# akuhara/RF_INV

Hardware: NVIDIA B200
Metric: forward+likelihood evals/sec (higher is better)
Workload: dtype f64

## Files before the change

### rf_inv_b200/csrc/forward.cu

```cuda
#include <cstdlib>
#include "rfinv_common.cuh"

#if defined(RFINV_PHASE_TIMING) && !defined(RFINV_FWD_GENERAL_TU)
__device__ unsigned long long g_phase[16];
#define PHASE_MARK(i)                                                            \
  do {                                                                           \
    if (tid == 0) {                                                              \
      const long long now__ = clock64();                                         \
      atomicAdd(&g_phase[i], (unsigned long long)(now__ - t_phase__));           \
      t_phase__ = now__;                                                         \
    }                                                                            \
  } while (0)
#define PHASE_INIT() long long t_phase__ = clock64(); if (tid == 0) atomicAdd(&g_phase[15], 1ULL)
extern "C" int rfinv_debug_get_phases(unsigned long long* out) {
  cudaError_t e = cudaMemcpyFromSymbol(out, g_phase, sizeof(g_phase));
  unsigned long long zero[16] = {0};
  cudaMemcpyToSymbol(g_phase, zero, sizeof(zero));
  return e == cudaSuccess ? 0 : 2;
}
#define PREP_MARK(i)                                                             \
  do {                                                                           \
    if (lane == 0) {                                                             \
      const long long now__ = clock64();                                         \
      atomicAdd(&g_phase[8 + (i)], (unsigned long long)(now__ - tp_phase__));    \
      tp_phase__ = now__;                                                        \
    }                                                                            \
  } while (0)
#define PREP_INIT() long long tp_phase__ = clock64()
#else
#define PHASE_MARK(i) do { } while (0)
#define PHASE_INIT() do { } while (0)
#define PREP_MARK(i) do { } while (0)
#define PREP_INIT() do { } while (0)
#endif

namespace {

struct LayerConst {
  double c1x, s1x, c1e, s1e;
  double c16x, s16x, c16e, s16e;
  double cbx, sbx, cbe, sbe;
  double t12, t21;
  double u11, u12, u21, u22;
  double cb2x, cb2e;
};
constexpr int LC_DOUBLES = sizeof(LayerConst) / sizeof(double);
static_assert(LC_DOUBLES % 2 == 0, "LayerConst is moved in 16-byte pieces");

struct TraceSel {
  int n;
  unsigned long long packed;
  __host__ __device__ int t(int i) const { return (int)((packed >> (4 * i)) & 15ULL); }
  __host__ void push(int trace) { packed |= (unsigned long long)trace << (4 * n); ++n; }
};
static_assert(RFINV_MAX_TRC <= 16, "TraceSel packs trace indices in four bits");

struct RayConst {
  double h14[4], h23[4];
  double a1, b1;
  double q1a, q1b, q2a, q2b;
  double thw, cbw, sbw;
  double wseed[4];
  double tp;
  double2 edge[4];
  double sta[4];
  int k, valid;
  int npre, l_sta;
};
constexpr int RC_DOUBLES = sizeof(RayConst) / sizeof(double);
static_assert(sizeof(RayConst) % 16 == 0, "RayConst is moved in 16-byte pieces");

__device__ __forceinline__ void rot(double& c, double& s, double cb, double sb) {
  double c2 = c * cb - s * sb;
  double s2 = s * cb + c * sb;
  c = c2;
  s = s2;
}

struct Wave { double a1, a2, b1, b2; };

__device__ __forceinline__ void wave_rotate(Wave& w, double c1, double s1, double c2, double s2) {
  const double a1 = fma(-s1, w.a2, c1 * w.a1);
  const double a2 = fma(s1, w.a1, c1 * w.a2);
  const double b1 = fma(-s2, w.b2, c2 * w.b1);
  const double b2 = fma(s2, w.b1, c2 * w.b2);
  w.a1 = a1; w.a2 = a2; w.b1 = b1; w.b2 = b2;
}

__device__ __forceinline__ void wave_interface(Wave& w, double t12, double t21, double u11, double u12, double u21,
                                               double u22) {
  const double a1 = fma(t12, w.b1, w.a1);
  const double b1 = fma(t21, w.a1, w.b1);
  const double a2 = fma(u12, w.b2, u11 * w.a2);
  const double b2 = fma(u22, w.b2, u21 * w.a2);
  w.a1 = a1; w.a2 = a2; w.b1 = b1; w.b2 = b2;
}

__device__ __forceinline__ double2 cmul(double2 a, double2 b) {
  return make_double2(a.x * b.x - a.y * b.y, a.x * b.y + a.y * b.x);
}

__device__ __forceinline__ void surface_response(const double* h14, const double* h23, const Wave& wa, const Wave& wb,
                                                 double cw, int ipha, double2& fr, double2& fv, double gain = 1.0) {
  const double2 A3 = make_double2(fma(h14[0], wa.a1, h14[1] * wa.b1), fma(h23[0], wa.a2, h23[1] * wa.b2));
  const double2 A4 = make_double2(fma(h14[2], wa.a1, h14[3] * wa.b1), fma(h23[2], wa.a2, h23[3] * wa.b2));
  const double2 B3 = make_double2(fma(h14[0], wb.a1, h14[1] * wb.b1), fma(h23[0], wb.a2, h23[1] * wb.b2));
  const double2 B4 = make_double2(fma(h14[2], wb.a1, h14[3] * wb.b1), fma(h23[2], wb.a2, h23[3] * wb.b2));
  const double2 p = cmul(A3, B4), q = cmul(B3, A4);
  const double2 dl = make_double2(p.x - q.x, p.y - q.y);
  const double rn = gain / (dl.x * dl.x + dl.y * dl.y);
  const double2 inv = make_double2(dl.x * rn, -dl.y * rn);
  double2 ur, uz;
  if (ipha >= 0) {
    ur = cmul(B4, inv);
    const double2 w = cmul(A4, inv);
    uz = make_double2(w.y * cw, -w.x * cw);
  } else {
    const double2 w0 = cmul(B3, inv);
    ur = make_double2(-w0.x, -w0.y);
    const double2 w = cmul(A3, inv);
    uz = make_double2(-w.y * cw, w.x * cw);
  }
  fr = make_double2(ur.x, -ur.y);
  fv = make_double2(-uz.x, uz.y);
}

__device__ __forceinline__ void surface_response_buried(const double* h14, const double* h23, const Wave& wa, const Wave& wb,
                                                        int ipha, double2 ya, double2 yb, double2& fr, double2& fv) {
  const double2 A3 = make_double2(fma(h14[0], wa.a1, h14[1] * wa.b1), fma(h23[0], wa.a2, h23[1] * wa.b2));
  const double2 A4 = make_double2(fma(h14[2], wa.a1, h14[3] * wa.b1), fma(h23[2], wa.a2, h23[3] * wa.b2));
  const double2 B3 = make_double2(fma(h14[0], wb.a1, h14[1] * wb.b1), fma(h23[0], wb.a2, h23[1] * wb.b2));
  const double2 B4 = make_double2(fma(h14[2], wb.a1, h14[3] * wb.b1), fma(h23[2], wb.a2, h23[3] * wb.b2));
  const double2 p = cmul(A3, B4), q = cmul(B3, A4);
  const double2 dl = make_double2(p.x - q.x, p.y - q.y);
  const double rn = 1.0 / (dl.x * dl.x + dl.y * dl.y);
  const double2 inv = make_double2(dl.x * rn, -dl.y * rn);
  double2 al, be;
  if (ipha >= 0) {
    al = cmul(B4, inv);
    const double2 w = cmul(A4, inv);
    be = make_double2(-w.x, -w.y);
  } else {
    const double2 w0 = cmul(B3, inv);
    al = make_double2(-w0.x, -w0.y);
    be = cmul(A3, inv);
  }
  const double2 ur = make_double2(fma(al.x, ya.x, be.x * yb.x), fma(al.y, ya.x, be.y * yb.x));
  const double2 s = make_double2(fma(al.x, ya.y, be.x * yb.y), fma(al.y, ya.y, be.y * yb.y));
  const double2 uz = make_double2(-s.y, s.x);
  fr = make_double2(ur.x, -ur.y);
  fv = make_double2(-uz.x, uz.y);
}

__device__ __forceinline__ void mat2_mul(const double* a, const double* b, double* c) {
  const double c0 = fma(a[0], b[0], a[1] * b[2]), c1 = fma(a[0], b[1], a[1] * b[3]);
  const double c2 = fma(a[2], b[0], a[3] * b[2]), c3 = fma(a[2], b[1], a[3] * b[3]);
  c[0] = c0; c[1] = c1; c[2] = c2; c[3] = c3;
}

struct PrepBasis {
  double v14[4], v23[4];
  double i14[4], i23[4];
};
struct PrepSerial {
  double tr[8];
  double ic[6];
  double tpterm, pad;
};
struct PrepShared {
  double h, rho, irho, beta2, inv_b2, inv_a2, a, b;
};
constexpr int PB_DOUBLES = sizeof(PrepBasis) / sizeof(double), PS_DOUBLES = sizeof(PrepSerial) / sizeof(double);
constexpr int PSH_DOUBLES = sizeof(PrepShared) / sizeof(double);
constexpr int PREP_RAYS_PER_PASS = 6;
constexpr int PREP_MISC_DOUBLES = 8;
__host__ __device__ inline size_t prep_sorted_doubles(int km) { return ((size_t)3 * km + 1) & ~(size_t)1; }
__host__ __device__ inline size_t prep_smem_model_doubles(int km) { return prep_sorted_doubles(km) + (size_t)(km + 2) * PSH_DOUBLES + PREP_MISC_DOUBLES; }
__host__ __device__ inline size_t prep_smem_ray_doubles(int km) { return (size_t)(km + 1) * PB_DOUBLES + (size_t)km * PS_DOUBLES + RC_DOUBLES + 8; }

__device__ __forceinline__ void small_sincos(double x, double* sn, double* cs) {
  if (fabs(x) < 0.01) {
    const double x2 = x * x;
    *cs = fma(x2, fma(x2, fma(x2, -1.0 / 720.0, 1.0 / 24.0), -0.5), 1.0);
    *sn = x * fma(x2, fma(x2, fma(x2, -1.0 / 5040.0, 1.0 / 120.0), -1.0 / 6.0), 1.0);
  } else {
    sincos(x, sn, cs);
  }
}

__device__ __forceinline__ double warp_scan_mul(double x, int lane) {
#pragma unroll
  for (int o = 1; o < 32; o <<= 1) {
    const double y = __shfl_up_sync(0xffffffffu, x, o);
    if (lane >= o) x *= y;
  }
  return x;
}

template <bool BURIED, bool HOSTLAYOUT>
__global__ void __maxnreg__(80) prep_kernel(const DevConfig cfg, const ModelBatch mb, double* __restrict__ lc_out,
                                                                 double* __restrict__ rc_out, uint8_t* __restrict__ is_valid,
                                                                 int* __restrict__ counter, int n_models, int ntr_eff, int nthr_fwd,
                                                                 int rays_per_cta, int m_begin) {
  extern __shared__ __align__(16) double prep_smem[];
  const int warp = threadIdx.x >> 5, lane = threadIdx.x & 31;
  const int n_groups = (ntr_eff + rays_per_cta - 1) / rays_per_cta;
  const int bm = blockIdx.x / n_groups, t_first = (blockIdx.x - bm * n_groups) * rays_per_cta;
  const int ci = m_begin + bm;
  const int nr_cta = min(rays_per_cta, ntr_eff - t_first);
  pdl_trigger();
  if (blockIdx.x == 0 && m_begin == 0 && threadIdx.x < RFINV_MAX_TRC) counter[threadIdx.x] = 0;
  if (ci >= n_models) return;
  if (mb.n_active_dev && ci >= *mb.n_active_dev) return;
  const int c = mb.active ? mb.active[ci] : ci;
  const int km = cfg.k_max, C = mb.C;
  const bool has_ray = warp < nr_cta;
  const int t0 = t_first + (has_ray ? warp : 0);
  const size_t item = (size_t)ci * ntr_eff + t0;
  double* zs = prep_smem;
  double *dps = zs + km, *dss = dps + km;
  PrepShared* LA = reinterpret_cast<PrepShared*>(zs + prep_sorted_doubles(km));
  double* s_misc = reinterpret_cast<double*>(LA + km + 2);
  int* s_int = reinterpret_cast<int*>(s_misc + 1);
  double* ray0 = s_misc + PREP_MISC_DOUBLES;
  const size_t ray_stride = prep_smem_ray_doubles(km);
  auto ray_basis = [&](int t) { return reinterpret_cast<PrepBasis*>(ray0 + (size_t)t * ray_stride); };
  auto ray_serial = [&](int t) { return reinterpret_cast<PrepSerial*>(ray0 + (size_t)t * ray_stride + (size_t)(km + 1) * PB_DOUBLES); };
  auto ray_const = [&](int t) { return reinterpret_cast<RayConst*>(ray0 + (size_t)t * ray_stride + (size_t)(km + 1) * PB_DOUBLES + (size_t)km * PS_DOUBLES); };
  auto ray_water = [&](int t) { return reinterpret_cast<double*>(ray_const(t)) + RC_DOUBLES; };
  constexpr bool buried = BURIED;

  PREP_INIT();
  if (warp == 0) {
    int k = mb.k[c];
    double zr[2] = {0.0, 0.0}, dr[2] = {0.0, 0.0}, sr[2] = {0.0, 0.0};
    static_assert(RFINV_MAX_K <= 64, "two elements per lane");
#pragma unroll
    for (int q = 0; q < 2; ++q) {
      const int i = lane + 32 * q;
      if (i < km - 1) {
        if (HOSTLAYOUT) {
          zr[q] = mb.z[(size_t)c * (km - 1) + i]; sr[q] = mb.dvs[(size_t)c * km + i];
          if (cfg.vp_mode == 1) dr[q] = mb.dvp[(size_t)c * km + i];
        } else {
          zr[q] = mb.z[(size_t)i * C + c]; dr[q] = mb.dvp[(size_t)i * C + c]; sr[q] = mb.dvs[(size_t)i * C + c];
        }
      }
    }
    double dvs_half, dvp_half = 0.0;
    if (HOSTLAYOUT) { dvs_half = mb.dvs[(size_t)c * km + km - 1]; if (cfg.vp_mode == 1) dvp_half = mb.dvp[(size_t)c * km + km - 1]; }
    else { dvs_half = mb.dvs[(size_t)(km - 1) * C + c]; dvp_half = mb.dvp[(size_t)(km - 1) * C + c]; }
    k = k < 1 ? 1 : (k > km - 1 ? km - 1 : k);
    double* zu = reinterpret_cast<double*>(ray_basis(0));
    double *du = zu + km, *su = du + km;
#pragma unroll
    for (int q = 0; q < 2; ++q) {
      const int i = lane + 32 * q;
      if (i < k) { zu[i] = zr[q]; du[i] = dr[q]; su[i] = sr[q]; }
    }
    __syncwarp();
    for (int i = lane; i < k; i += 32) {
      const double zi = zu[i];
      int rank = 0;
      for (int j = 0; j < k; ++j) { const double zj = zu[j]; rank += (zj < zi || (zj == zi && j < i)) ? 1 : 0; }
      zs[rank] = zi; dps[rank] = du[i]; dss[rank] = su[i];
    }
    __syncwarp();

    int ls = -1;
    double h_part = 0.0;
    if (buried) {
      double z_tmp = 0.0;
      ls = k;
      for (int l = 0; l < k; ++l) {
        const double hl = l == 0 ? __dsub_rn(zs[0], cfg.sdep) : __dsub_rn(zs[l], zs[l - 1]);
        z_tmp = __dadd_rn(z_tmp, hl);
        if (!(z_tmp < cfg.bdep)) { ls = l; h_part = __dsub_rn(__dadd_rn(cfg.bdep, hl), z_tmp); break; }
      }
      if (ls == k) h_part = __dsub_rn(cfg.bdep, z_tmp);
    }
    const int ka = buried ? k + 1 : k;
    PREP_MARK(0);
    bool valid = true;
    for (int la = lane; la <= ka; la += 32) {
      const int l = (buried && la > ls) ? la - 1 : la;
      double zc, h, dvs_l, dvp_l;
      if (l == 0) { zc = __dmul_rn(0.5, __dadd_rn(cfg.sdep, zs[0])); h = __dsub_rn(zs[0], cfg.sdep); dvs_l = dss[0]; dvp_l = dps[0]; }
      else if (l < k) { zc = __dmul_rn(0.5, __dadd_rn(zs[l], zs[l - 1])); h = __dsub_rn(zs[l], zs[l - 1]); dvs_l = dss[l]; dvp_l = dps[l]; }
      else { zc = __dmul_rn(0.5, __dadd_rn(cfg.z_max, zs[k - 1])); h = 999.0; dvs_l = dvs_half; dvp_l = dvp_half; }
      double a, b;
      bool ok = layer_velocity(cfg, zc, dvs_l, dvp_l, a, b);
      if (l == 0) ok = ok && !(h < __dmul_rn(0.125, a));
      else if (l < k) ok = ok && !(h < cfg.h_min);
      valid = valid && ok;
      if (buried) {
        if (la == ls) h = h_part;
        else if (la == ls + 1 && ls < k) h = __dsub_rn(h, h_part);
      }
      PrepShared S;
      S.h = h; S.a = a; S.b = b;
      S.rho = vp_to_rho(a);
      S.irho = 1.0 / S.rho;
      S.beta2 = __dmul_rn(b, b);
      S.inv_b2 = __ddiv_rn(1.0, S.beta2);
      S.inv_a2 = __ddiv_rn(1.0, __dmul_rn(a, a));
      LA[la] = S;
    }
    valid = __all_sync(0xffffffffu, valid);
    if (lane == 0) { s_int[0] = k; s_int[1] = ls; s_int[2] = valid ? 1 : 0; s_misc[0] = h_part; }
    PREP_MARK(1);
  }
  __syncthreads();

  const int k = s_int[0], ls = s_int[1];
  const bool valid = s_int[2] != 0;
  const int ka = buried ? k + 1 : k;
  const int kb = (buried && ls == k) ? k : ka;
  PrepBasis* PB = ray_basis(warp);
  PrepSerial* PS = ray_serial(warp);
  if (has_ray) {

  const double p = cfg.rayp[t0];
  const int ipha = cfg.ipha[t0];
  const double p2 = __dmul_rn(p, p);
  const double nyq = (double)(cfg.nfft / 2);
  int nyq_doublings = 0;
  while ((nthr_fwd << nyq_doublings) < cfg.nfft_p2 / 2) ++nyq_doublings;
  for (int la = lane; la <= ka; la += 32) {
    const PrepShared S = LA[la];
    const double h = S.h, rho = S.rho, beta2 = S.beta2;
    double tp_sign = 1.0;
    if (buried) {
      if (la == ls) tp_sign = ls == k ? -1.0 : 0.0;
      else if (la < ls) tp_sign = 0.0;
    }
    const double bp = 1.0 - 2.0 * beta2 * p2;
    const double eta = sqrt(__dsub_rn(S.inv_b2, p2));
    const double xi = sqrt(__dsub_rn(S.inv_a2, p2));
    if (la < ka) {
      PrepBasis& Q = PB[la];
      PrepSerial& Z = PS[la];
      const double g2 = 2.0 * beta2 * p;
      const double ieta = 1.0 / eta, irho = S.irho, ixi = 1.0 / xi;
      Q.v14[0] = p; Q.v14[1] = 1.0; Q.v14[2] = rho * bp; Q.v14[3] = -rho * g2;
      Q.v23[0] = xi; Q.v23[1] = -p * ieta; Q.v23[2] = -rho * g2 * xi; Q.v23[3] = -rho * bp * ieta;
      Q.i14[0] = g2; Q.i14[1] = irho; Q.i14[2] = bp; Q.i14[3] = -p * irho;
      Q.i23[0] = bp * ixi; Q.i23[1] = -p * irho * ixi; Q.i23[2] = -g2 * eta; Q.i23[3] = -eta * irho;
      Z.tpterm = cfg.deconv_mode == 0 ? __dmul_rn(tp_sign, __dmul_rn(h, ipha == 1 ? xi : eta)) : 0.0;
      LayerConst* L = reinterpret_cast<LayerConst*>(lc_out) + item * km + la;
      const double thx = cfg.domg * xi * h, the = cfg.domg * eta * h;
      double snx, csx, sne, cse;
      sincos(thx, &snx, &csx); L->c1x = csx; L->s1x = snx;
      sincos(the, &sne, &cse); L->c1e = cse; L->s1e = sne;
#pragma unroll
      for (int d = 0; d < 4; ++d) {
        const double c2 = fma(csx, csx, -snx * snx), s2 = 2.0 * csx * snx; csx = c2; snx = s2;
        const double c3 = fma(cse, cse, -sne * sne), s3 = 2.0 * cse * sne; cse = c3; sne = s3;
      }
      L->c16x = csx; L->s16x = snx; L->c16e = cse; L->s16e = sne;
      for (int b = 16; b < nthr_fwd; b <<= 1) {
        const double c2 = fma(csx, csx, -snx * snx), s2 = 2.0 * csx * snx; csx = c2; snx = s2;
        const double c3 = fma(cse, cse, -sne * sne), s3 = 2.0 * cse * sne; cse = c3; sne = s3;
      }
      L->cbx = csx; L->sbx = snx; L->cbe = cse; L->sbe = sne;
      L->cb2x = csx + csx; L->cb2e = cse + cse;
      small_sincos((double)1.0e-5f * xi * h, &Z.tr[1], &Z.tr[0]);
      small_sincos((double)1.0e-5f * eta * h, &Z.tr[3], &Z.tr[2]);
      double cn = csx, sn2 = snx, ce = cse, se = sne;
      if (cfg.fft_general) {
        sincos(nyq * thx, &sn2, &cn);
        sincos(nyq * the, &se, &ce);
      } else {
        for (int d = 0; d < nyq_doublings; ++d) {
          const double c2 = fma(cn, cn, -sn2 * sn2), s2 = 2.0 * cn * sn2; cn = c2; sn2 = s2;
          const double c3 = fma(ce, ce, -se * se), s3 = 2.0 * ce * se; ce = c3; se = s3;
        }
      }
      Z.tr[4] = cn; Z.tr[5] = sn2; Z.tr[6] = ce; Z.tr[7] = se;
    } else {
      double* W = ray_water(warp);
      W[4] = xi; W[5] = eta; W[6] = bp;
    }
  }
  __syncwarp();

  PREP_MARK(2);
  double carryP = 1.0, carryS = 1.0;
  double sP_last = 1.0, sS_last = 1.0;
  double sP_sta = 1.0, sS_sta = 1.0;
  for (int base = 0; base < ka; base += 32) {
    const int l = base + lane;
    double t14[4] = {1.0, 0.0, 0.0, 1.0}, t23[4] = {1.0, 0.0, 0.0, 1.0};
    if (l >= 1 && l < ka) {
      mat2_mul(PB[l].i14, PB[l - 1].v14, t14);
      mat2_mul(PB[l].i23, PB[l - 1].v23, t23);
    }
    const double sP = carryP * warp_scan_mul(t14[0], lane), sS = carryS * warp_scan_mul(t14[3], lane);
    double sPp = __shfl_up_sync(0xffffffffu, sP, 1), sSp = __shfl_up_sync(0xffffffffu, sS, 1);
    if (lane == 0) { sPp = carryP; sSp = carryS; }
    if (l >= 1 && l < ka) {
      double* ic = PS[l - 1].ic;
      const double rP = 1.0 / sP, rS = 1.0 / sS;
      const double pp = sPp * rP, sp = sSp * rP, ps = sPp * rS, ss = sSp * rS;
      ic[0] = t14[1] * sp; ic[1] = t14[2] * ps;
      ic[2] = t23[0] * pp; ic[3] = t23[1] * sp; ic[4] = t23[2] * ps; ic[5] = t23[3] * ss;
      LayerConst* L = reinterpret_cast<LayerConst*>(lc_out) + item * km + (l - 1);
      L->t12 = ic[0]; L->t21 = ic[1]; L->u11 = ic[2]; L->u12 = ic[3]; L->u21 = ic[4]; L->u22 = ic[5];
    }
    const int last_lane = (ka - 1 - base) < 31 ? (ka - 1 - base) : 31;
    if (buried && ls >= base && ls < base + 32) { sP_sta = __shfl_sync(0xffffffffu, sP, ls - base); sS_sta = __shfl_sync(0xffffffffu, sS, ls - base); }
    if (kb - 1 >= base && kb - 1 < base + 32) { sP_last = __shfl_sync(0xffffffffu, sP, kb - 1 - base); sS_last = __shfl_sync(0xffffffffu, sS, kb - 1 - base); }
    carryP = __shfl_sync(0xffffffffu, sP, last_lane);
    carryS = __shfl_sync(0xffffffffu, sS, last_lane);
  }
  if (lane == 0) {
    LayerConst* L = reinterpret_cast<LayerConst*>(lc_out) + item * km + (ka - 1);
    L->t12 = 0.0; L->t21 = 0.0; L->u11 = 1.0; L->u12 = 0.0; L->u21 = 0.0; L->u22 = 1.0;
    double* ic = PS[ka - 1].ic;
    ic[0] = 0.0; ic[1] = 0.0; ic[2] = 1.0; ic[3] = 0.0; ic[4] = 0.0; ic[5] = 1.0;
  }
  __syncwarp();

  PREP_MARK(3);
  {
    RayConst R;
    double cw0 = 1.0, sw0 = 0.0, cw1 = 1.0, sw1 = 0.0, rw = 0.0;
    if (cfg.sdep > 0.0) {
      const double aw = 1.5, rhow = 1.0, hw = cfg.sdep;
      const double xiw = sqrt(1.0 / (aw * aw) - p * p);
      R.thw = cfg.domg * xiw * hw;
      sincos(R.thw, &R.wseed[1], &R.wseed[0]);
      R.cbw = R.wseed[0]; R.sbw = R.wseed[1];
#pragma unroll
      for (int d = 0; d < 4; ++d) { const double c2 = fma(R.cbw, R.cbw, -R.sbw * R.sbw), s2 = 2.0 * R.cbw * R.sbw; R.cbw = c2; R.sbw = s2; }
      R.wseed[2] = R.cbw; R.wseed[3] = R.sbw;
      for (int b = 16; b < nthr_fwd; b <<= 1) { const double c2 = fma(R.cbw, R.cbw, -R.sbw * R.sbw), s2 = 2.0 * R.cbw * R.sbw; R.cbw = c2; R.sbw = s2; }
      rw = rhow / xiw;
      small_sincos((double)1.0e-5f * xiw * hw, &sw0, &cw0);
      sincos(nyq * R.thw, &sw1, &cw1);
    } else {
      R.thw = 0.0; R.cbw = 1.0; R.sbw = 0.0;
      R.wseed[0] = R.wseed[2] = 1.0; R.wseed[1] = R.wseed[3] = 0.0;
    }
    {
      const PrepShared& H = LA[ka];
      const double* W = ray_water(warp);
      const double a = H.a, b = H.b, rho = H.rho, beta2 = H.beta2, xi = W[4], eta = W[5], bp = W[6];
      const double r1 = 1.0 / (2.0 * rho * a * xi), r2 = 1.0 / (2.0 * rho * b * eta);
      const double e11 = beta2 * p * (2.0 * rho * xi) * r1, e12 = bp * rho * r1, e13 = p * r1, e14 = xi * r1;
      const double e21 = bp * rho * r2, e22 = b * p, e23 = eta * r2, e24 = p * r2;
      const double r14[4] = {e11, e14, e21, -e24};
      const double r23[4] = {-e12, e13, e22, e23};
      const PrepBasis& Q = PB[kb - 1];
      const double v14[4] = {Q.v14[0] * sP_last, Q.v14[1] * sS_last, Q.v14[2] * sP_last, Q.v14[3] * sS_last};
      const double v23[4] = {Q.v23[0] * sP_last, Q.v23[1] * sS_last, Q.v23[2] * sP_last, Q.v23[3] * sS_last};
      mat2_mul(r14, v14, R.h14);
      mat2_mul(r23, v23, R.h23);
    }
    {
      const PrepBasis& Q = PB[0];
      R.a1 = Q.i14[0]; R.b1 = Q.i14[2];
      R.q1a = -rw * Q.i14[1]; R.q1b = -rw * Q.i14[3];
      R.q2a = Q.i23[0]; R.q2b = Q.i23[2];
    }
    R.l_sta = -1;
    R.sta[0] = R.sta[1] = R.sta[2] = R.sta[3] = 0.0;
    if (buried) {
      const PrepBasis& Q = PB[ls];
      R.l_sta = ls;
      R.sta[0] = Q.v14[0] * sP_sta; R.sta[1] = Q.v14[1] * sS_sta;
      R.sta[2] = Q.v23[0] * sP_sta; R.sta[3] = Q.v23[1] * sS_sta;
    }
    R.k = kb;
    R.valid = valid;
    R.tp = 0.0; R.npre = 0;
#pragma unroll
    for (int i = 0; i < 4; ++i) R.edge[i] = make_double2(0.0, 0.0);
    if (lane == 0) {
      *ray_const(warp) = R;
      double* W = ray_water(warp);
      W[0] = cw0; W[1] = sw0; W[2] = cw1; W[3] = sw1;
    }
  }
  PREP_MARK(4);
  }
  __syncthreads();

  for (int r0 = warp * PREP_RAYS_PER_PASS; r0 < nr_cta; r0 += (int)(blockDim.x >> 5) * PREP_RAYS_PER_PASS) {
    const int nr = min(PREP_RAYS_PER_PASS, nr_cta - r0);
    const bool vec_lane = lane < 4 * nr, tp_lane = lane >= 4 * nr && lane < 5 * nr;
    const int tr_ray = r0 + (vec_lane ? (lane >> 2) : (tp_lane ? lane - 4 * nr : 0));
    const RayConst* Rr = ray_const(tr_ray);
    const double* Wr = ray_water(tr_ray);
    const PrepSerial* Zr = ray_serial(tr_ray);
    const bool is_b = lane & 1, is_nyq = (lane >> 1) & 1;
    Wave w;
    double2 y_sta = make_double2(0.0, 0.0);
    double tp = 0.0;
    {
      const double cw = is_nyq ? Wr[2] : Wr[0], sw = is_nyq ? Wr[3] : Wr[1];
      if (!is_b) { w.a1 = Rr->a1; w.b1 = Rr->b1; w.a2 = 0.0; w.b2 = 0.0; }
      else { w.a1 = sw * Rr->q1a; w.b1 = sw * Rr->q1b; w.a2 = cw * Rr->q2a; w.b2 = cw * Rr->q2b; }
    }
    if (vec_lane) {
      const int o = is_nyq ? 4 : 0;
      const double st0 = Rr->sta[0], st1 = Rr->sta[1], st2 = Rr->sta[2], st3 = Rr->sta[3];
      Wave w_bc = w;
      for (int l = 0; l < ka; ++l) {
        const PrepSerial& Q = Zr[l];
        wave_rotate(w, Q.tr[o], Q.tr[o + 1], Q.tr[o + 2], Q.tr[o + 3]);
        if (buried && l == ls) { y_sta.x = fma(st0, w.a1, st1 * w.b1); y_sta.y = fma(st2, w.a2, st3 * w.b2); }
        if (l == kb - 1) w_bc = w;
        if (l + 1 < ka) wave_interface(w, Q.ic[0], Q.ic[1], Q.ic[2], Q.ic[3], Q.ic[4], Q.ic[5]);
      }
      w = w_bc;
    } else if (tp_lane) {
      for (int l = 0; l < ka; ++l) tp = __dadd_rn(tp, Zr[l].tpterm);
      RayConst* Rw = ray_const(tr_ray);
      const int iph = cfg.ipha[t_first + tr_ray];
      Rw->tp = tp;
      Rw->npre = iph == 1 ? f_nint((-cfg.t_start - tp) / cfg.delta)
                          : f_nint((-cfg.t_start + tp) / cfg.delta);
    }
    PREP_MARK(5);
    {
      const int rr = lane >> 1, e = lane & 1;
      const bool fin = lane < 2 * nr;
      const int src_a = fin ? 4 * rr + 2 * e : 0, src_b = src_a + 1;
      Wave ea, eb;
      ea.a1 = __shfl_sync(0xffffffffu, w.a1, src_a); ea.a2 = __shfl_sync(0xffffffffu, w.a2, src_a);
      ea.b1 = __shfl_sync(0xffffffffu, w.b1, src_a); ea.b2 = __shfl_sync(0xffffffffu, w.b2, src_a);
      eb.a1 = __shfl_sync(0xffffffffu, w.a1, src_b); eb.a2 = __shfl_sync(0xffffffffu, w.a2, src_b);
      eb.b1 = __shfl_sync(0xffffffffu, w.b1, src_b); eb.b2 = __shfl_sync(0xffffffffu, w.b2, src_b);
      const double2 ya = make_double2(__shfl_sync(0xffffffffu, y_sta.x, src_a), __shfl_sync(0xffffffffu, y_sta.y, src_a));
      const double2 yb = make_double2(__shfl_sync(0xffffffffu, y_sta.x, src_b), __shfl_sync(0xffffffffu, y_sta.y, src_b));
      if (fin) {
        RayConst* Rf = ray_const(r0 + rr);
        const double* Wf = ray_water(r0 + rr);
        double h14[4], h23[4];
#pragma unroll
        for (int i = 0; i < 4; ++i) { h14[i] = Rf->h14[i]; h23[i] = Rf->h23[i]; }
        double2 fr, fv;
        if (!buried) surface_response(h14, h23, ea, eb, e ? Wf[2] : Wf[0], cfg.ipha[t_first + r0 + rr], fr, fv);
        else surface_response_buried(h14, h23, ea, eb, cfg.ipha[t_first + r0 + rr], ya, yb, fr, fv);
        Rf->edge[2 * e] = fr; Rf->edge[2 * e + 1] = fv;
      }
    }
  }
  __syncthreads();
  {
    double2* dst = reinterpret_cast<double2*>(rc_out + ((size_t)ci * ntr_eff + t_first) * RC_DOUBLES);
    for (int i = threadIdx.x; i < nr_cta * (RC_DOUBLES / 2); i += blockDim.x) {
      const int t = i / (RC_DOUBLES / 2), j = i - t * (RC_DOUBLES / 2);
      dst[i] = reinterpret_cast<const double2*>(ray_const(t))[j];
    }
    if (is_valid && threadIdx.x == 0 && t_first == 0) is_valid[c] = (uint8_t)valid;
  }
  PREP_MARK(6);
}

__host__ __device__ inline size_t fft_twiddle_entries(size_t n) {
  size_t e = 0;
  for (size_t N = n; N > 8; N >>= 3) e += 7 * (N >> 3);
  return e;
}
__device__ __forceinline__ void fill_fft_twiddles(double2* s_tw, const double2* __restrict__ tw, int n, int tid, int nthr) {
  int off = 0;
  for (int N = n; N > 8; N >>= 3) {
    const int stride = N >> 3, tmul = n / N;
    for (int i = tid; i < 7 * stride; i += nthr) {
      const int q = i / stride + 1, o = i - (q - 1) * stride;
      s_tw[off + i] = tw[q * o * tmul];
    }
    off += 7 * stride;
  }
}

__host__ __device__ __forceinline__ int fft_pad_shift(int log2n) { return log2n >= 9 ? log2n - 3 : 31; }
__device__ __forceinline__ int fpad(int p, int sh) { return p + (p >> 3) + (p >> sh); }
__device__ __forceinline__ unsigned fpad(unsigned p, int sh) { return p + (p >> 3) + (p >> sh); }
__host__ __device__ inline size_t fft_buf_elems(size_t n) { return n + (n >> 3) + 9; }

template <bool ZA, bool ZB>
__device__ __forceinline__ double2 zadd(double2 a, double2 b) {
  if constexpr (ZA && ZB) return make_double2(0.0, 0.0);
  else if constexpr (ZB) return a;
  else if constexpr (ZA) return b;
  else return make_double2(a.x + b.x, a.y + b.y);
}
template <bool ZA, bool ZB>
__device__ __forceinline__ double2 zsub(double2 a, double2 b) {
  if constexpr (ZA && ZB) return make_double2(0.0, 0.0);
  else if constexpr (ZB) return a;
  else if constexpr (ZA) return make_double2(-b.x, -b.y);
  else return make_double2(a.x - b.x, a.y - b.y);
}
template <unsigned Z = 0u>
__device__ __forceinline__ void dft8(double2* v) {
  const double hs = 0.70710678118654752440;
  constexpr bool z0 = Z & 1u, z1 = Z & 2u, z2 = Z & 4u, z3 = Z & 8u, z4 = Z & 16u, z5 = Z & 32u, z6 = Z & 64u, z7 = Z & 128u;
  double2 e0, e1, e2, e3, o0, o1, o2, o3;
  {
    const double2 a = zadd<z0, z4>(v[0], v[4]), b = zsub<z0, z4>(v[0], v[4]);
    const double2 c = zadd<z2, z6>(v[2], v[6]), dd = zsub<z2, z6>(v[2], v[6]), d = make_double2(-dd.y, dd.x);
    e0 = make_double2(a.x + c.x, a.y + c.y); e1 = make_double2(b.x + d.x, b.y + d.y);
    e2 = make_double2(a.x - c.x, a.y - c.y); e3 = make_double2(b.x - d.x, b.y - d.y);
  }
  {
    const double2 a = zadd<z1, z5>(v[1], v[5]), b = zsub<z1, z5>(v[1], v[5]);
    const double2 c = zadd<z3, z7>(v[3], v[7]), dd = zsub<z3, z7>(v[3], v[7]), d = make_double2(-dd.y, dd.x);
    o0 = make_double2(a.x + c.x, a.y + c.y);
    const double2 t1 = make_double2(b.x + d.x, b.y + d.y), t2 = make_double2(a.x - c.x, a.y - c.y);
    const double2 t3 = make_double2(b.x - d.x, b.y - d.y);
    o1 = make_double2((t1.x - t1.y) * hs, (t1.x + t1.y) * hs);
    o2 = make_double2(-t2.y, t2.x);
    o3 = make_double2(-(t3.x + t3.y) * hs, (t3.x - t3.y) * hs);
  }
  v[0] = make_double2(e0.x + o0.x, e0.y + o0.y); v[4] = make_double2(e0.x - o0.x, e0.y - o0.y);
  v[1] = make_double2(e1.x + o1.x, e1.y + o1.y); v[5] = make_double2(e1.x - o1.x, e1.y - o1.y);
  v[2] = make_double2(e2.x + o2.x, e2.y + o2.y); v[6] = make_double2(e2.x - o2.x, e2.y - o2.y);
  v[3] = make_double2(e3.x + o3.x, e3.y + o3.y); v[7] = make_double2(e3.x - o3.x, e3.y - o3.y);
}

struct CtaSync { __device__ __forceinline__ void operator()() const { __syncthreads(); } };
__device__ __forceinline__ void publish_max(double v, double* s_red, int tid) {
  for (int o = 16; o > 0; o >>= 1) v = fmax(v, __shfl_xor_sync(0xffffffffu, v, o));
  if ((tid & 31) == 0) s_red[tid >> 5] = v;
}

template <int LOG2N, int N, class Sync, int PLO = 8, int PHI = -1, bool WL = false>
__device__ __forceinline__ void fft_stage8(double2* buf, const double2* __restrict__ stw, double& vmax, double* s_red, int tid,
                                           int nthr, Sync sync) {
  constexpr unsigned n = 1u << LOG2N, stride = N >> 3;
  constexpr bool prune = PLO <= PHI;
  constexpr unsigned zmask = prune ? (((1u << (PHI + 1)) - 1u) & ~((1u << PLO) - 1u)) : 0u;
  constexpr int PSH = LOG2N >= 9 ? LOG2N - 3 : 31;
  constexpr bool last = (N == 8);
  for (unsigned j = tid; j < (n >> 3); j += nthr) {
    const unsigned o = j & (stride - 1), base = ((j - o) << 3) + o;
    double2 v[8];
    unsigned pos[8];
    if (stride % 8 == 0) {
      const unsigned p0 = fpad(base, PSH);
      constexpr unsigned step = stride + (stride >> 3) + (PSH < 31 ? (stride >> PSH) : 0u);
#pragma unroll
      for (int r = 0; r < 8; ++r) pos[r] = p0 + r * step;
    } else {
#pragma unroll
      for (int r = 0; r < 8; ++r) pos[r] = fpad(base + r * stride, PSH);
    }
#pragma unroll
    for (int r = 0; r < 8; ++r) if (!((zmask >> r) & 1u)) v[r] = buf[pos[r]];
    if (!last) {
      double2 w[7];
#pragma unroll
      for (int q = 1; q < 8; ++q) w[q - 1] = stw[(q - 1) * stride + o];
      dft8<zmask>(v);
      if (prune && o == 0) {
        const double2 x = buf[pos[4]];
#pragma unroll
        for (int q = 0; q < 8; ++q) v[q] = (q & 1) ? make_double2(v[q].x - x.x, v[q].y - x.y) : make_double2(v[q].x + x.x, v[q].y + x.y);
      }
#pragma unroll
      for (int q = 1; q < 8; ++q) v[q] = cmul(v[q], w[q - 1]);
    } else {
      dft8(v);
#pragma unroll
      for (int q = 0; q < 8; ++q) vmax = fmax(vmax, v[q].y);
    }
    buf[pos[0]] = v[0]; buf[pos[4]] = v[1]; buf[pos[2]] = v[2]; buf[pos[6]] = v[3];
    buf[pos[1]] = v[4]; buf[pos[5]] = v[5]; buf[pos[3]] = v[6]; buf[pos[7]] = v[7];
  }
  if (last) publish_max(vmax, s_red, tid);
  if constexpr (WL && N < (1 << LOG2N) && !(last && LOG2N % 3 == 0)) __syncwarp();
  else sync();
  if constexpr (N >= 64) fft_stage8<LOG2N, (N >> 3), Sync, 8, -1, WL>(buf, stw + 7 * stride, vmax, s_red, tid, nthr, sync);
}

template <int LOG2N, class Sync, int JP = 0, int NT = 1>
__device__ __forceinline__ double fft_inverse_dif_n(double2* buf, const double2* twq, double* s_red, int tid, int nthr, Sync sync) {
  constexpr unsigned n = 1u << LOG2N;
#ifdef RFINV_NO_FFT_PRUNE
  constexpr int PLO = 8, PHI = -1;
#else
  constexpr int jfull = (1 << (LOG2N - 1)) / NT;
  constexpr int PLO = (JP > 0 && LOG2N >= 6) ? (4 * JP + jfull - 1) / jfull : 8, PHI = 7 - PLO;
#endif
  constexpr int PSH = LOG2N >= 9 ? LOG2N - 3 : 31;
  constexpr int REM = LOG2N % 3;
#ifdef RFINV_NO_FFT_WARPLOCAL
  constexpr bool WL = false;
#else
  constexpr bool WL = NT >= 32 && (NT << 3) == (1 << LOG2N) && LOG2N >= 9;
#endif
  double vmax = -INFINITY;
  fft_stage8<LOG2N, (1 << LOG2N), Sync, PLO, PHI, WL>(buf, twq, vmax, s_red, tid, nthr, sync);
  if (REM == 2) {
    for (unsigned jj = tid; jj < (n >> 2); jj += nthr) {
      const unsigned j = WL ? (((unsigned)tid >> 5) << 6) + ((unsigned)tid & 31u) + ((jj >= (unsigned)nthr) ? 32u : 0u) : jj;
      const unsigned p0 = fpad(j << 2, PSH);
      const double2 v0 = buf[p0], v1 = buf[p0 + 1], v2 = buf[p0 + 2], v3 = buf[p0 + 3];
      const double2 a0 = make_double2(v0.x + v2.x, v0.y + v2.y), a1 = make_double2(v0.x - v2.x, v0.y - v2.y);
      const double2 a2 = make_double2(v1.x + v3.x, v1.y + v3.y), a3 = make_double2(-(v1.y - v3.y), v1.x - v3.x);
      const double2 r0 = make_double2(a0.x + a2.x, a0.y + a2.y), r1 = make_double2(a1.x + a3.x, a1.y + a3.y);
      const double2 r2 = make_double2(a0.x - a2.x, a0.y - a2.y), r3 = make_double2(a1.x - a3.x, a1.y - a3.y);
      vmax = fmax(fmax(vmax, r0.y), fmax(fmax(r1.y, r2.y), r3.y));
      buf[p0] = r0; buf[p0 + 2] = r1; buf[p0 + 1] = r2; buf[p0 + 3] = r3;
    }
    publish_max(vmax, s_red, tid);
    sync();
  } else if (REM == 1) {
    for (unsigned jj = tid, i = 0; jj < (n >> 1); jj += nthr, ++i) {
      const unsigned j = WL ? (((unsigned)tid >> 5) << 7) + ((unsigned)tid & 31u) + 32u * i : jj;
      const unsigned p0 = fpad(j << 1, PSH);
      const double2 a = buf[p0], b = buf[p0 + 1];
      const double2 r0 = make_double2(a.x + b.x, a.y + b.y), r1 = make_double2(a.x - b.x, a.y - b.y);
      vmax = fmax(vmax, fmax(r0.y, r1.y));
      buf[p0] = r0; buf[p0 + 1] = r1;
    }
    publish_max(vmax, s_red, tid);
    sync();
  }
  const int nw = (nthr + 31) >> 5;
  double r = s_red[0];
  for (int i = 1; i < nw; ++i) r = fmax(r, s_red[i]);
  return r;
}

template <int LO, int HI, class Sync, int JP = 0, int NT = 1>
__device__ __forceinline__ double fft_inverse_dif(double2* buf, int n, const double2* twq, double* s_red, int tid, int nthr, Sync sync) {
  if constexpr (LO == HI) {
    return fft_inverse_dif_n<LO, Sync, JP, NT>(buf, twq, s_red, tid, nthr, sync);
  } else {
    if (n == (1 << LO)) return fft_inverse_dif_n<LO, Sync, JP, NT>(buf, twq, s_red, tid, nthr, sync);
    return fft_inverse_dif<LO + 1, HI, Sync, JP, NT>(buf, n, twq, s_red, tid, nthr, sync);
  }
}

template <int LOG2M, class Sync>
__device__ __forceinline__ double bluestein_inverse_m(double2* buf, int n, const double2* __restrict__ chirp,
                                                      const double2* __restrict__ chirp_b, const double2* twq, double* s_red,
                                                      int tid, int nthr, Sync sync) {
  constexpr unsigned M = 1u << LOG2M;
  constexpr int PSH = LOG2M >= 9 ? LOG2M - 3 : 31;
  fft_inverse_dif_n<LOG2M, Sync>(buf, twq, s_red, tid, nthr, sync);
  for (unsigned p = tid; p < M; p += nthr) {
    const unsigned q = __brev(p) >> (32 - LOG2M);
    if (p > q) continue;
    const double2 u = buf[fpad(p, PSH)], v = buf[fpad(q, PSH)];
    const double2 bq = chirp_b[q], bp = chirp_b[p];
    buf[fpad(q, PSH)] = cmul(make_double2(u.x, -u.y), bq);
    if (p != q) buf[fpad(p, PSH)] = cmul(make_double2(v.x, -v.y), bp);
  }
  sync();
  fft_inverse_dif_n<LOG2M, Sync>(buf, twq, s_red, tid, nthr, sync);
  double vmax = -INFINITY;
  for (unsigned p = tid; p < M; p += nthr) {
    const unsigned q = __brev(p) >> (32 - LOG2M);
    if (p > q) continue;
    const double2 u = buf[fpad(p, PSH)], v = buf[fpad(q, PSH)];
    if (q < (unsigned)n) { const double2 x = cmul(u, chirp[q]); buf[fpad(q, PSH)] = x; vmax = fmax(vmax, x.y); }
    if (p != q && p < (unsigned)n) { const double2 x = cmul(v, chirp[p]); buf[fpad(p, PSH)] = x; vmax = fmax(vmax, x.y); }
  }
  publish_max(vmax, s_red + 32, tid);
  sync();
  const int nw = (nthr + 31) >> 5;
  double r = s_red[32];
  for (int i = 1; i < nw; ++i) r = fmax(r, s_red[32 + i]);
  return r;
}
template <int LO, int HI, class Sync>
__device__ __forceinline__ double bluestein_inverse(double2* buf, const DevConfig& cfg, const double2* twq, double* s_red, int tid,
                                                    int nthr, Sync sync) {
  if constexpr (LO == HI) {
    return bluestein_inverse_m<LO, Sync>(buf, cfg.nfft, cfg.chirp, cfg.chirp_b, twq, s_red, tid, nthr, sync);
  } else {
    if (cfg.log2n == LO) return bluestein_inverse_m<LO, Sync>(buf, cfg.nfft, cfg.chirp, cfg.chirp_b, twq, s_red, tid, nthr, sync);
    return bluestein_inverse<LO + 1, HI, Sync>(buf, cfg, twq, s_red, tid, nthr, sync);
  }
}

template <class Sync>
__device__ __forceinline__ double block_max(double v, double* scratch, int tid, int nthr, Sync sync) {
  for (int o = 16; o > 0; o >>= 1) v = fmax(v, __shfl_xor_sync(0xffffffffu, v, o));
  sync();
  if ((tid & 31) == 0) scratch[tid >> 5] = v;
  sync();
  const int nw = (nthr + 31) >> 5;
  double r = scratch[0];
  for (int i = 1; i < nw; ++i) r = fmax(r, scratch[i]);
  return r;
}

__device__ __forceinline__ void cp_async16(void* smem_dst, const void* gmem_src) {
  const unsigned d = (unsigned)__cvta_generic_to_shared(smem_dst);
  asm volatile("cp.async.cg.shared.global [%0], [%1], 16;\n" ::"r"(d), "l"(gmem_src));
}

__host__ __device__ inline size_t trig_table_entries(size_t km, size_t nthr) { return (16 + (nthr >> 4)) * (2 * km + 1); }
template <int NT>
__device__ __forceinline__ void build_trig_tables(double2* s_tab, const LayerConst* s_lc, int k, int km, int tid) {
  constexpr int n_hi = NT >> 4;
  const int ts = 2 * km + 1;
  for (int task = tid; task < 4 * k; task += NT) {
    const int level = task >= 2 * k ? 1 : 0, idx = task - level * 2 * k;
    const int l = idx >> 1, which = idx & 1;
    double2* dst = s_tab + (level ? 16 * ts : 0) + idx;
    double2 e[16];
    e[0] = make_double2(1.0, 0.0);
    e[1] = reinterpret_cast<const double2*>(&s_lc[l].c1x)[2 * level + which];
#pragma unroll
    for (int len = 2; len < 16; len <<= 1) {
      e[len] = e[len >> 1];
      rot(e[len].x, e[len].y, e[len >> 1].x, e[len >> 1].y);
#pragma unroll
      for (int j = 1; j < len; ++j) {
        e[len + j] = e[j];
        rot(e[len + j].x, e[len + j].y, e[len].x, e[len].y);
      }
    }
#pragma unroll
    for (int i = 0; i < 16; ++i)
      if (i < n_hi || !level) dst[i * ts] = e[i];
  }
}

__device__ __forceinline__ void build_water_table(double2* s_tabw, const RayConst* s_rc, int n_hi, int tid, int nthr) {
  const int level = nthr - 1 - tid;
  if (level > 1 || s_rc->thw == 0.0) return;
  const int cnt = level ? n_hi : 16;
  double2 e[16];
  e[0] = make_double2(1.0, 0.0);
  e[1] = make_double2(s_rc->wseed[2 * level], s_rc->wseed[2 * level + 1]);
#pragma unroll
  for (int len = 2; len < 16; len <<= 1) {
    e[len] = e[len >> 1];
    rot(e[len].x, e[len].y, e[len >> 1].x, e[len >> 1].y);
#pragma unroll
    for (int j = 1; j < len; ++j) {
      e[len + j] = e[j];
      rot(e[len + j].x, e[len + j].y, e[len].x, e[len].y);
    }
  }
#pragma unroll
  for (int i = 0; i < 16; ++i)
    if (i < cnt) s_tabw[level * 16 + i] = e[i];
}
__device__ __forceinline__ void water_phase(const double2* s_tabw, double thw, int tid, double& cw, double& sw) {
  cw = 1.0; sw = 0.0;
  if (thw != 0.0) {
    const double2 a = s_tabw[tid & 15], b = s_tabw[16 + (tid >> 4)];
    cw = a.x; sw = a.y;
    rot(cw, sw, b.x, b.y);
  }
}

template <int J, int NT>
__device__ __forceinline__ void propagate(const RayConst* s_rc, const LayerConst* s_lc, const double2* s_tab, const double2* s_tabw,
                                          int k, int km, int tid, Wave* wa, Wave* wb) {
  {
    const double thw = s_rc->thw, cbw = s_rc->cbw, sbw = s_rc->sbw;
    const double a1 = s_rc->a1, b1 = s_rc->b1, q1a = s_rc->q1a, q1b = s_rc->q1b, q2a = s_rc->q2a, q2b = s_rc->q2b;
    double cw, sw;
    water_phase(s_tabw, thw, tid, cw, sw);
#pragma unroll
    for (int m = 0; m < J; ++m) {
      wa[m].a1 = a1; wa[m].a2 = 0.0; wa[m].b1 = b1; wa[m].b2 = 0.0;
      wb[m].a1 = sw * q1a; wb[m].b1 = sw * q1b; wb[m].a2 = cw * q2a; wb[m].b2 = cw * q2b;
      rot(cw, sw, cbw, sbw);
    }
  }
  const int ts = 2 * km + 1;
  const double2* p_lo = s_tab + (tid & 15) * ts;
  const double2* p_hi = s_tab + (16 + (tid >> 4)) * ts;
  double c1, s1, c2, s2;
  {
    const double2 a = p_lo[0], cc = p_lo[1], b = p_hi[0], d = p_hi[1];
    c1 = a.x; s1 = a.y; rot(c1, s1, b.x, b.y);
    c2 = cc.x; s2 = cc.y; rot(c2, s2, d.x, d.y);
  }
  for (int l = 0; l < k; ++l) {
    const LayerConst& L = s_lc[l];
    const int ln = l + 1 < k ? l + 1 : l;
    double2 na, ncc, nb, nd;
    double pc1 = 0.0, ps1 = 0.0, pc2 = 0.0, ps2 = 0.0;
    auto advance = [&](int m) {
      if (m == 0) {
        pc1 = c1; ps1 = s1; pc2 = c2; ps2 = s2;
        rot(c1, s1, L.cbx, L.sbx);
        rot(c2, s2, L.cbe, L.sbe);
      } else {
        const double cb2x = L.cb2x, cb2e = L.cb2e;
        const double n1 = fma(cb2x, c1, -pc1), m1 = fma(cb2x, s1, -ps1), n2 = fma(cb2e, c2, -pc2), m2 = fma(cb2e, s2, -ps2);
        pc1 = c1; ps1 = s1; pc2 = c2; ps2 = s2;
        c1 = n1; s1 = m1; c2 = n2; s2 = m2;
      }
    };
    if (l + 1 < k) {
      const double t12 = L.t12, t21 = L.t21, u11 = L.u11, u12 = L.u12, u21 = L.u21, u22 = L.u22;
#pragma unroll
      for (int m = 0; m < J; ++m) {
#ifndef RFINV_NO_TABPREFETCH
        if (m == J - 1) { na = p_lo[2 * ln]; ncc = p_lo[2 * ln + 1]; nb = p_hi[2 * ln]; nd = p_hi[2 * ln + 1]; }
#endif
        wave_rotate(wa[m], c1, s1, c2, s2);
        wave_rotate(wb[m], c1, s1, c2, s2);
        wave_interface(wa[m], t12, t21, u11, u12, u21, u22);
        wave_interface(wb[m], t12, t21, u11, u12, u21, u22);
        if (m + 1 < J) advance(m);
      }
#ifdef RFINV_NO_TABPREFETCH
      na = p_lo[2 * ln]; ncc = p_lo[2 * ln + 1]; nb = p_hi[2 * ln]; nd = p_hi[2 * ln + 1];
#endif
      c1 = na.x; s1 = na.y; rot(c1, s1, nb.x, nb.y);
      c2 = ncc.x; s2 = ncc.y; rot(c2, s2, nd.x, nd.y);
    } else {
#pragma unroll
      for (int m = 0; m < J; ++m) {
        wave_rotate(wa[m], c1, s1, c2, s2);
        wave_rotate(wb[m], c1, s1, c2, s2);
        if (m + 1 < J) advance(m);
      }
    }
  }
}

template <int JB, int NT, bool MIXED>
__device__ __forceinline__ void propagate_groups(int jm, const RayConst* s_rc, const LayerConst* s_lc, const double2* s_tab,
                                                 const double2* s_tabw, int k, int km, int tid, Wave* wa, Wave* wb) {
  if (!MIXED || jm >= JB) { propagate<JB, NT>(s_rc, s_lc, s_tab, s_tabw, k, km, tid, wa, wb); return; }
  if constexpr (MIXED) {
  if constexpr (JB > 6) if (jm == 6) { propagate<6, NT>(s_rc, s_lc, s_tab, s_tabw, k, km, tid, wa, wb); return; }
  if constexpr (JB > 4) if (jm == 4) { propagate<4, NT>(s_rc, s_lc, s_tab, s_tabw, k, km, tid, wa, wb); return; }
  if constexpr (JB > 3) if (jm == 3) { propagate<3, NT>(s_rc, s_lc, s_tab, s_tabw, k, km, tid, wa, wb); return; }
  if constexpr (JB > 2) if (jm == 2) { propagate<2, NT>(s_rc, s_lc, s_tab, s_tabw, k, km, tid, wa, wb); return; }
  if constexpr (JB > 1) propagate<1, NT>(s_rc, s_lc, s_tab, s_tabw, k, km, tid, wa, wb);
  }
}

template <int J, bool STAGE, bool GEN>
__device__ __forceinline__ void surface_and_pack(const RayConst* s_rc, const Wave* wa, const Wave* wb, int jfull, int ipha,
                                                 int n, int nh, int tid, int nthr, const double* __restrict__ flt, double2* s_buf,
                                                 double2* s_fr, double2* s_fv, bool buried, const double2* s_tabw, int psh,
                                                 const double2* __restrict__ chirp = nullptr, int fft_len = 0) {
  const bool odd = GEN && (n & 1);
  const int jtop = odd ? nh : nh - 1;
  const double wsgn = odd ? -1.0 : 1.0;
  double h14[4], h23[4];
#pragma unroll
  for (int i = 0; i < 4; ++i) { h14[i] = s_rc->h14[i]; h23[i] = s_rc->h23[i]; }
  const double thw = s_rc->thw, cbw = s_rc->cbw, sbw = s_rc->sbw;
  double cw, sw;
  water_phase(s_tabw, thw, tid, cw, sw);
#pragma unroll
  for (int m = 0; m < J; ++m) {
    const int j = tid + m * nthr;
    double2 fr, fv;
    const bool live = !GEN || j < jtop;
    if (STAGE && buried) { if (live) surface_response_buried(h14, h23, wa[m], wb[m], ipha, s_fr[j], s_fv[j], fr, fv); }
    else surface_response(h14, h23, wa[m], wb[m], cw, ipha, fr, fv, STAGE ? 1.0 : (live ? flt[j] : 0.0));
    rot(cw, sw, cbw, sbw);
    if (STAGE) {
      if (j > 0 && live) { s_fr[j] = fr; s_fv[j] = fv; }
    } else if (GEN) {
      if (j > 0 && live) {
        const double2 xv = fv;
        const double2 xr = ipha == 1 ? fr : xv;
        const double2 w = chirp[j];
        const double2 a = cmul(make_double2(xr.x - xv.y, xr.y + xv.x), w);
        const double2 b = cmul(make_double2(xr.x + xv.y, xv.x - xr.y), w);
        s_buf[fpad(j, psh)] = make_double2(a.x, -a.y);
        s_buf[fpad(n - j, psh)] = make_double2(wsgn * b.x, -wsgn * b.y);
      }
    } else if (j > 0) {
      const double2 xv = fv;
      const double2 xr = ipha == 1 ? fr : xv;
      s_buf[fpad(j, psh)] = make_double2(xr.x - xv.y, xr.y + xv.x);
      s_buf[fpad(n - j, psh)] = make_double2(xr.x + xv.y, xv.x - xr.y);
    }
  }
  for (int m = J; m < jfull; ++m) {
    const int j = tid + m * nthr;
    if (GEN && j >= jtop) continue;
    if (STAGE) { s_fr[j] = make_double2(0.0, 0.0); s_fv[j] = make_double2(0.0, 0.0); }
    else { s_buf[fpad(j, psh)] = make_double2(0.0, 0.0); s_buf[fpad(n - j, psh)] = make_double2(0.0, 0.0); }
  }
  if (GEN && !STAGE) for (int f = n + tid; f < fft_len; f += nthr) s_buf[fpad(f, psh)] = make_double2(0.0, 0.0);
  if (!GEN && !STAGE && tid == 0 && 2 * jfull * nthr < n) {
    s_buf[fpad(jfull * nthr, psh)] = make_double2(0.0, 0.0);
    s_buf[fpad(n - jfull * nthr, psh)] = make_double2(0.0, 0.0);
  }
  if (tid == 0) {
    if (STAGE) {
      s_fr[0] = s_rc->edge[0]; s_fv[0] = s_rc->edge[1];
      if (!odd) { s_fr[nh - 1] = s_rc->edge[2]; s_fv[nh - 1] = s_rc->edge[3]; }
    } else {
      const double f0 = flt[0], f1 = flt[nh - 1];
      const double2 r0 = ipha == 1 ? s_rc->edge[0] : s_rc->edge[1], r1 = ipha == 1 ? s_rc->edge[2] : s_rc->edge[3];
      if (GEN) {
        s_buf[fpad(0, psh)] = make_double2(r0.x * f0, -s_rc->edge[1].x * f0);
        if (!odd) {
          const double2 a = cmul(make_double2(r1.x * f1, s_rc->edge[3].x * f1), chirp[nh - 1]);
          s_buf[fpad(nh - 1, psh)] = make_double2(a.x, -a.y);
        }
      } else {
        s_buf[fpad(0, psh)] = make_double2(r0.x * f0, s_rc->edge[1].x * f0);
        s_buf[fpad(nh - 1, psh)] = make_double2(r1.x * f1, s_rc->edge[3].x * f1);
      }
    }
  }
}

constexpr int OBS_PRE = 4;
__device__ __forceinline__ int obs_pre_index(int S, int q, int tid, int nthr) {
  const int pr = tid + (q >> 1) * nthr;
  return pr < (S >> 1) ? ((q & 1) ? S - 1 - pr : pr) : S;
}
template <bool GEN>
__device__ __forceinline__ void write_outputs(const DevConfig& cfg, const EvalOutputs& out, const double2* s_buf, int C, int c,
                                              int t, int ipha, int npre, double scale, const double* obs_pre, int tid, int nthr) {
  const int n = cfg.nfft, S = cfg.nsmp, Sp = cfg.nsmp_pad, nmask = n - 1, brev_shift = 32 - cfg.log2n, psh = fft_pad_shift(cfg.log2n);
  double* __restrict__ mis = out.misfit + ((size_t)t * C + c) * Sp;
  double* smp_base = out.rft_smp;
  if (out.slot && ((out.slot[c] ^ out.slot_invert) & 1)) smp_base = out.rft_smp_alt;
  double* __restrict__ smp = smp_base ? smp_base + ((size_t)t * C + c) * S : nullptr;
  const double* __restrict__ obs = cfg.obs + (size_t)t * S;
  auto sample = [&](int i) {
    if constexpr (GEN) {
      int f = (ipha == 1 ? i - npre : npre - i - 1) % n;
      if (f < 0) f += n;
      const double v = s_buf[fpad(f, psh)].x * scale;
      return ipha == 1 ? v : -v;
    }
    const int f = ipha == 1 ? ((i - npre) & nmask)
                            : ((npre - i - 1) & nmask);
    const double v = s_buf[fpad((int)(__brev((unsigned)f) >> brev_shift), psh)].x * scale;
    return ipha == 1 ? v : -v;
  };
  const bool split = cfg.qf_split[t] != 0;
  const int ha = S >> 1, half = Sp >> 1;
  auto emit = [&](int pr, double o1, double o2) {
    const double v1 = sample(pr), v2 = sample(S - 1 - pr);
    const double d1 = v1 - o1, d2 = v2 - o2;
    mis[pr] = split ? d1 + d2 : d1;
    mis[split ? half + pr : S - 1 - pr] = split ? d1 - d2 : d2;
    if (smp) { smp[pr] = v1; smp[S - 1 - pr] = v2; }
  };
#pragma unroll
  for (int q = 0; q < OBS_PRE / 2; ++q) {
    const int pr = tid + q * nthr;
    if (pr < ha) emit(pr, obs_pre[2 * q], obs_pre[2 * q + 1]);
  }
  for (int pr = tid + (OBS_PRE / 2) * nthr; pr < ha; pr += nthr) emit(pr, __ldg(obs + pr), __ldg(obs + S - 1 - pr));
  if ((S & 1) && tid == 0) {
    const double v = sample(ha);
    mis[ha] = v - __ldg(obs + ha);
    if (smp) smp[ha] = v;
  }
  if (split) {
    for (int i = S - ha + tid; i < half; i += nthr) mis[i] = 0.0;
    for (int i = half + ha + tid; i < Sp; i += nthr) mis[i] = 0.0;
  } else {
    for (int i = S + tid; i < Sp; i += nthr) mis[i] = 0.0;
  }
  if (out.rft_full) {
    double* __restrict__ full = out.rft_full + ((size_t)c * cfg.ntrc + t) * n;
    for (int i = tid; i < n; i += nthr) full[i] = sample(i);
  }
}

template <int JB, bool STAGE, bool MIXED, bool GEN>
__device__ __forceinline__ void surface_groups(int jm, const RayConst* s_rc, const Wave* wa, const Wave* wb, int jfull, int ipha, int n,
                                               int nh, int tid, int nthr, const double* __restrict__ flt, double2* s_buf,
                                               double2* s_fr, double2* s_fv, bool buried, const double2* s_tabw, int psh,
                                               const double2* __restrict__ chirp, int fft_len) {
#define SURF(JM) surface_and_pack<JM, STAGE, GEN>(s_rc, wa, wb, jfull, ipha, n, nh, tid, nthr, flt, s_buf, s_fr, s_fv, buried, s_tabw, psh, chirp, fft_len)
  if (!MIXED || jm >= JB) { SURF(JB); return; }
  if constexpr (MIXED) {
  if constexpr (JB > 6) if (jm == 6) { SURF(6); return; }
  if constexpr (JB > 4) if (jm == 4) { SURF(4); return; }
  if constexpr (JB > 3) if (jm == 3) { SURF(3); return; }
  if constexpr (JB > 2) if (jm == 2) { SURF(2); return; }
  if constexpr (JB > 1) SURF(1);
  }
#undef SURF
}

template <int J, int BMAX, int MINB, bool MIXED, bool BURIED, bool GEN = false>
__global__ void __launch_bounds__(BMAX, MINB) forward_kernel(const DevConfig cfg, const ModelBatch mb, const EvalOutputs out,
                                                             const double* __restrict__ lc_in,
                                                             const double* __restrict__ rc_in, int* __restrict__ counter,
                                                             const TraceSel sel) {
  extern __shared__ __align__(16) unsigned char smem_raw[];
  __shared__ int s_next;
  const int tid = threadIdx.x;
  constexpr int nthr = BMAX;
  const int n = cfg.nfft, nh = cfg.nh, km = cfg.k_max, C = mb.C, psh = fft_pad_shift(cfg.log2n);
  const int ntr_eff = cfg.ray_common ? 1 : cfg.ntrc;
  constexpr bool buried = BURIED;
  const bool general = cfg.ray_common || cfg.deconv_mode == 1 || buried;

  constexpr int n_hi = nthr >> 4;
  const int nf = GEN ? cfg.fft_len : n;
  const size_t tab_entries = trig_table_entries(km, nthr);
  const size_t region0 = tab_entries > fft_buf_elems(nf) ? tab_entries : fft_buf_elems(nf);
  double2* s_buf = reinterpret_cast<double2*>(smem_raw);
  double2* s_tab = s_buf;
  double2* s_fr = s_buf + region0;
  double2* s_fv = s_fr + (nh + 1);
  double2* s_twq_sm = s_fr + (general ? 2 * (nh + 1) : 0);
  const double2* s_twq = GEN ? cfg.twq : s_twq_sm;
  double* s_red = reinterpret_cast<double*>(s_twq_sm + (GEN ? 0 : fft_twiddle_entries(nf)));
  RayConst* s_rc2 = reinterpret_cast<RayConst*>(s_red + 64);
  LayerConst* s_lc2 = reinterpret_cast<LayerConst*>(s_rc2 + 2);
  double2* s_tabw = reinterpret_cast<double2*>(s_lc2 + 2 * (size_t)km);

  const unsigned sel_magic = sel.n > 1 ? (unsigned)((0x100000000ULL + (unsigned)sel.n - 1u) / (unsigned)sel.n) : 0u;
  auto div_sel = [&](int x) { return sel.n > 1 ? (int)__umulhi((unsigned)x, sel_magic) : x; };
  auto prefetch = [&](int item_sel, int slot) {
    const int ci_ = div_sel(item_sel);
    const size_t item = (size_t)ci_ * ntr_eff + sel.t(item_sel - ci_ * sel.n);
    const double2* src = reinterpret_cast<const double2*>(rc_in + (size_t)item * RC_DOUBLES);
    double2* dst = reinterpret_cast<double2*>(s_rc2 + slot);
    for (int i = tid; i < RC_DOUBLES / 2; i += nthr) cp_async16(dst + i, src + i);
    const double2* src2 = reinterpret_cast<const double2*>(lc_in + (size_t)item * km * LC_DOUBLES);
    double2* dst2 = reinterpret_cast<double2*>(s_lc2 + (size_t)slot * km);
    for (int i = tid; i < km * (LC_DOUBLES / 2); i += nthr) cp_async16(dst2 + i, src2 + i);
  };

  int item = blockIdx.x, slot = 0;
  pdl_trigger();
  if (!GEN) fill_fft_twiddles(s_twq_sm, cfg.tw, nf, tid, nthr);
  pdl_wait();
  const int n_items = (mb.n_active_dev ? *mb.n_active_dev : (mb.active ? mb.n_active : C)) * sel.n;
  if (item >= n_items) return;
  prefetch(item, 0);
  asm volatile("cp.async.commit_group;\n" ::);
  if (tid == 0) s_next = (int)gridDim.x + atomicAdd(counter, 1);
  asm volatile("cp.async.wait_all;\n" ::);
  __syncthreads();

  while (item < n_items) {
    PHASE_INIT();
    const int next = s_next;
    if (next < n_items) prefetch(next, slot ^ 1);
    asm volatile("cp.async.commit_group;\n" ::);
    int next2 = 0;
    if (tid == 0) next2 = atomicAdd(counter, 1);
    const RayConst* s_rc = s_rc2 + slot;
    const LayerConst* s_lc = s_lc2 + (size_t)slot * km;
    const int ci = div_sel(item), t0 = sel.t(item - ci * sel.n);
    const int c = mb.active ? mb.active[ci] : ci;
    const int k = s_rc->k;
    const int ipha = cfg.ipha[t0];
    PHASE_MARK(0);
    build_trig_tables<nthr>(s_tab, s_lc, buried ? max(k, s_rc->l_sta + 1) : k, km, tid);
    build_water_table(s_tabw, s_rc, n_hi, tid, nthr);
    __syncthreads();
    PHASE_MARK(1);

    const int jm = MIXED ? cfg.jbins[t0] : J;
    Wave wa[J], wb[J];
    for (int pass = buried ? 0 : 1; pass < 2; ++pass) {
      propagate_groups<J, nthr, MIXED>(jm, s_rc, s_lc, s_tab, s_tabw, pass == 0 ? s_rc->l_sta + 1 : k, km, tid, wa, wb);
      if (pass == 0) {
        const double c0 = s_rc->sta[0], c1 = s_rc->sta[1], c2 = s_rc->sta[2], c3 = s_rc->sta[3];
#pragma unroll
        for (int m = 0; m < J; ++m) {
          const int j = tid + m * nthr;
          if (m < jm && (!GEN || j < nh)) {
            s_fr[j] = make_double2(fma(c0, wa[m].a1, c1 * wa[m].b1), fma(c2, wa[m].a2, c3 * wa[m].b2));
            s_fv[j] = make_double2(fma(c0, wb[m].a1, c1 * wb[m].b1), fma(c2, wb[m].a2, c3 * wb[m].b2));
          }
        }
      }
    }
    PHASE_MARK(2);
    __syncthreads();

    const int jfull = (cfg.nfft_p2 >> 1) / nthr;
#ifdef RFINV_NO_FFT_PRUNE
    constexpr bool kPruned = false;
#else
    constexpr bool kPruned = !GEN;
#endif
    if (general) surface_groups<J, true, MIXED, GEN>(jm, s_rc, wa, wb, jfull, ipha, n, nh, tid, nthr, nullptr, s_buf, s_fr, s_fv, buried, s_tabw, psh, cfg.chirp, nf);
    else surface_groups<J, false, MIXED, GEN>(jm, s_rc, wa, wb, kPruned ? J : jfull, ipha, n, nh, tid, nthr, cfg.flt + (size_t)t0 * nh, s_buf, s_fr, s_fv, false, s_tabw, psh, cfg.chirp, nf);
    __syncthreads();
    PHASE_MARK(3);

    if (cfg.deconv_mode == 1) {
      const double2* xs = ipha == 1 ? s_fv : s_fr;
      const double2* ys = ipha == 1 ? s_fr : s_fv;
      double mx = -INFINITY;
      for (int j = tid; j < nh; j += nthr) mx = fmax(mx, xs[j].x * xs[j].x + xs[j].y * xs[j].y);
      mx = block_max(mx, s_red, tid, nthr, CtaSync());
      const double wlvl = 0.001 * mx;
      double2 keep[J + 1];
#pragma unroll
      for (int q = 0; q < J + 1; ++q) {
        const int j = tid + q * nthr;
        if (j < nh) {
          const double2 x = xs[j], y = ys[j];
          const double amp = x.x * x.x + x.y * x.y;
          const double d = fmax(amp, wlvl);
          keep[q] = make_double2((y.x * x.x + y.y * x.y) / d, (y.y * x.x - y.x * x.y) / d);
        }
      }
      __syncthreads();
#pragma unroll
      for (int q = 0; q < J + 1; ++q) {
        const int j = tid + q * nthr;
        if (j < nh) s_fr[j] = keep[q];
      }
      __syncthreads();
    }

    const int t_begin = cfg.ray_common ? 0 : t0, t_end = cfg.ray_common ? cfg.ntrc : t0 + 1;
    for (int t = t_begin; t < t_end; ++t) {
      if (general) {
        const double* __restrict__ flt = cfg.flt + (size_t)t * nh;
        const double2* src_r = (cfg.deconv_mode == 1 || ipha == 1) ? s_fr : s_fv;
        for (int j = tid; j < nh; j += nthr) {
          const double f = flt[j];
          const double2 xr = make_double2(src_r[j].x * f, src_r[j].y * f);
          double2 xv = make_double2(0.0, 0.0);
          if (cfg.deconv_mode == 0) xv = make_double2(s_fv[j].x * f, s_fv[j].y * f);
          const bool edge_bin = j == 0 || (j == nh - 1 && !(GEN && (n & 1)));
          if constexpr (GEN) {
            const double2 w = cfg.chirp[j];
            if (edge_bin) {
              const double2 a = cmul(make_double2(xr.x, xv.x), w);
              s_buf[fpad(j, psh)] = make_double2(a.x, -a.y);
            } else {
              const double sg = (n & 1) ? -1.0 : 1.0;
              const double2 a = cmul(make_double2(xr.x - xv.y, xr.y + xv.x), w), b = cmul(make_double2(xr.x + xv.y, xv.x - xr.y), w);
              s_buf[fpad(j, psh)] = make_double2(a.x, -a.y);
              s_buf[fpad(n - j, psh)] = make_double2(sg * b.x, -sg * b.y);
            }
          } else if (edge_bin) {
            s_buf[fpad(j, psh)] = make_double2(xr.x, xv.x);
          } else {
            s_buf[fpad(j, psh)] = make_double2(xr.x - xv.y, xr.y + xv.x);
            s_buf[fpad(n - j, psh)] = make_double2(xr.x + xv.y, xv.x - xr.y);
          }
        }
        if constexpr (GEN) for (int f = n + tid; f < nf; f += nthr) s_buf[fpad(f, psh)] = make_double2(0.0, 0.0);
        __syncthreads();
      }
      PHASE_MARK(4);
      double obs_pre[OBS_PRE];
      const double* __restrict__ obs_t = cfg.obs + (size_t)t * cfg.nsmp;
#pragma unroll
      for (int q = 0; q < OBS_PRE; ++q) {
        const int i = obs_pre_index(cfg.nsmp, q, tid, nthr);
        obs_pre[q] = i < cfg.nsmp ? __ldg(obs_t + i) : 0.0;
      }
      constexpr int FLO = BMAX <= 32 ? 6 : (BMAX <= 64 ? 8 : (BMAX <= 128 ? 10 : 11));
      constexpr int FHI = BMAX <= 32 ? 7 : (BMAX <= 64 ? 9 : (BMAX <= 128 ? 10 : 12));
      double mx;
      if constexpr (GEN) mx = bluestein_inverse<FLO + 1, (FHI + 1 > 12 ? 12 : FHI + 1), CtaSync>(s_buf, cfg, s_twq, s_red, tid, nthr, CtaSync());
      else mx = fft_inverse_dif<FLO, FHI, CtaSync, J, nthr>(s_buf, n, s_twq, s_red, tid, nthr, CtaSync());
      PHASE_MARK(5);
      const double scale = cfg.deconv_mode == 0 ? 1.0 / mx : 1.0;
      write_outputs<GEN>(cfg, out, s_buf, C, c, t, ipha, s_rc->npre, scale, obs_pre, tid, nthr);
      if (tid == 0 && t + 1 == t_end) s_next = (int)gridDim.x + next2;
      asm volatile("cp.async.wait_all;\n" ::);
      __syncthreads();
      PHASE_MARK(6);
    }
    item = next;
    slot ^= 1;
  }
}

template <bool GEN>
__global__ void __launch_bounds__(128) filter_traces_kernel(const DevConfig cfg, const double* __restrict__ in,
                                                           const int* __restrict__ trace_of, double* __restrict__ out) {
  extern __shared__ __align__(16) unsigned char smem_raw[];
  const int tid = threadIdx.x, nthr = blockDim.x, n = cfg.nfft, nh = cfg.nh, brev_shift = 32 - cfg.log2n, psh = fft_pad_shift(cfg.log2n);
  const int nf = cfg.fft_len;
  double2* b0 = reinterpret_cast<double2*>(smem_raw);
  double2* b1 = b0 + fft_buf_elems(nf);
  double2* s_tw_sm = b1 + fft_buf_elems(nf);
  const double2* s_tw = GEN ? cfg.twq : s_tw_sm;
  double* s_red = reinterpret_cast<double*>(s_tw_sm + (GEN ? 0 : fft_twiddle_entries(nf)));
  const double* x = in + (size_t)blockIdx.x * n;
  const double* __restrict__ flt = cfg.flt + (size_t)trace_of[blockIdx.x] * nh;
  if (!GEN) fill_fft_twiddles(s_tw_sm, cfg.tw, nf, tid, nthr);
  if constexpr (GEN) {
    const bool odd = n & 1;
    for (int i = tid; i < nf; i += nthr) {
      double2 v = make_double2(0.0, 0.0);
      if (i < n) { const double2 w = cfg.chirp[i]; const double xi = x[i]; v = make_double2(xi * w.x, -xi * w.y); }
      b0[fpad(i, psh)] = v;
      if (i >= n) b1[fpad(i, psh)] = v;
    }
    __syncthreads();
    bluestein_inverse<7, 12>(b0, cfg, s_tw, s_red, tid, nthr, CtaSync());
    for (int f = tid; f < nh; f += nthr) {
      const double2 v = b0[fpad(f, psh)];
      const double g = flt[f];
      const double2 w = cfg.chirp[f];
      const bool edge_bin = f == 0 || (f == nh - 1 && !odd);
      double2 y = make_double2(v.x * g, -v.y * g);
      if (edge_bin) y.y = 0.0;
      const double2 a = cmul(y, w);
      b1[fpad(f, psh)] = make_double2(a.x, -a.y);
      if (!edge_bin) {
        const double sg = odd ? -1.0 : 1.0;
        const double2 b = cmul(make_double2(y.x, -y.y), w);
        b1[fpad(n - f, psh)] = make_double2(sg * b.x, -sg * b.y);
      }
    }
    __syncthreads();
    bluestein_inverse<7, 12>(b1, cfg, s_tw, s_red, tid, nthr, CtaSync());
    for (int i = tid; i < n; i += nthr) out[(size_t)blockIdx.x * n + i] = b1[fpad(i, psh)].x;
  } else {
  for (int i = tid; i < n; i += nthr) b0[fpad(i, psh)] = make_double2(x[i], 0.0);
  __syncthreads();
  fft_inverse_dif<6, 12>(b0, n, s_tw, s_red, tid, nthr, CtaSync());
  for (int f = tid; f < nh; f += nthr) {
    const double2 v = b0[fpad((int)(__brev((unsigned)f) >> brev_shift), psh)];
    const double w = flt[f];
    const double2 y = make_double2(v.x * w, -v.y * w);
    if (f == 0 || f == nh - 1) {
      b1[fpad(f, psh)] = make_double2(y.x, 0.0);
    } else {
      b1[fpad(f, psh)] = y;
      b1[fpad(n - f, psh)] = make_double2(y.x, -y.y);
    }
  }
  __syncthreads();
  fft_inverse_dif<6, 12>(b1, n, s_tw, s_red, tid, nthr, CtaSync());
  for (int i = tid; i < n; i += nthr) out[(size_t)blockIdx.x * n + i] = b1[fpad((int)(__brev((unsigned)i) >> brev_shift), psh)].x;
  }
}

__global__ void format_model_kernel(const DevConfig cfg, const ModelBatch mb, int* nlay_out, double* alpha,
                                    double* beta, double* rho, double* h, uint8_t* is_valid) {
  const int c = blockIdx.x * blockDim.x + threadIdx.x;
  if (c >= mb.C) return;
  const int km = cfg.k_max, C = mb.C, k = mb.k[c], stride = km + 1;
  double z[RFINV_MAX_K], dp[RFINV_MAX_K], ds[RFINV_MAX_K];
  for (int i = 0; i < k; ++i) {
    z[i] = mb.z[(size_t)i * C + c]; dp[i] = mb.dvp[(size_t)i * C + c]; ds[i] = mb.dvs[(size_t)i * C + c];
  }
  for (int i = 1; i < k; ++i) {
    const double a = z[i], b = dp[i], d = ds[i];
    int m = i - 1;
    while (m >= 0 && z[m] > a) { z[m + 1] = z[m]; dp[m + 1] = dp[m]; ds[m + 1] = ds[m]; --m; }
    z[m + 1] = a; dp[m + 1] = b; ds[m + 1] = d;
  }
  int i = 0;
  bool valid = true;
  double* A = alpha + (size_t)c * stride; double* Bt = beta + (size_t)c * stride;
  double* R = rho + (size_t)c * stride; double* H = h + (size_t)c * stride;
  if (cfg.sdep > 0.0) { A[i] = 1.5; Bt[i] = -999.0; R[i] = 1.0; H[i] = cfg.sdep; ++i; }
  for (int l = 0; l <= k; ++l) {
    double zc, hh, dvs_l, dvp_l;
    if (l == 0) { zc = __dmul_rn(0.5, __dadd_rn(cfg.sdep, z[0])); hh = __dsub_rn(z[0], cfg.sdep); dvs_l = ds[0]; dvp_l = dp[0]; }
    else if (l < k) { zc = __dmul_rn(0.5, __dadd_rn(z[l], z[l - 1])); hh = __dsub_rn(z[l], z[l - 1]); dvs_l = ds[l]; dvp_l = dp[l]; }
    else { zc = __dmul_rn(0.5, __dadd_rn(cfg.z_max, z[k - 1])); hh = 999.0;
           dvs_l = mb.dvs[(size_t)(km - 1) * C + c]; dvp_l = mb.dvp[(size_t)(km - 1) * C + c]; }
    double a, b;
    bool ok = layer_velocity(cfg, zc, dvs_l, dvp_l, a, b);
    if (l == 0) ok = ok && !(hh < __dmul_rn(0.125, a));
    else if (l < k) ok = ok && !(hh < cfg.h_min);
    valid = valid && ok;
    if (i < stride) { A[i] = a; Bt[i] = b; R[i] = vp_to_rho(a); H[i] = hh; }
    ++i;
  }
  nlay_out[c] = i;
  is_valid[c] = (uint8_t)valid;
}

size_t forward_smem_bytes(const DevConfig& cfg, int nthr) {
  const size_t n = cfg.fft_len, nh = cfg.nh, km = cfg.k_max;
  const size_t tab_entries = trig_table_entries(km, nthr);
  const size_t region0 = tab_entries > fft_buf_elems(n) ? tab_entries : fft_buf_elems(n);
  const bool general = cfg.ray_common || cfg.deconv_mode == 1 || cfg.bdep > 0.0;
  const size_t spectra = general ? 2 * (nh + 1) : 0;
  return sizeof(double2) * (region0 + spectra + (cfg.fft_general ? 0 : fft_twiddle_entries(n))) + sizeof(double) * 64 + 2 * sizeof(RayConst) +
         2 * sizeof(LayerConst) * km + sizeof(double2) * (16 + (nthr >> 4));
}

template <int J, int BMAX, int MINB, bool MIXED, bool BURIED, bool GEN = false>
int launch_forward_t(const DevConfig& cfg, const ModelBatch& mb, const EvalOutputs& out, const double* lc,
                     const double* rc, int* counter, int nthr, cudaStream_t stream, const TraceSel& sel) {
  static const size_t extra = getenv("RFINV_FWD_EXTRA_SMEM") ? (size_t)atoi(getenv("RFINV_FWD_EXTRA_SMEM")) : 0;
  const size_t smem = forward_smem_bytes(cfg, nthr) + extra;
  if (nthr != BMAX) { rfinv_set_error("forward_kernel<%d,%d>: launched with %d threads", J, BMAX, nthr); return RFINV_ERR_ARG; }
  RFINV_CUDA_CHECK(rfinv_raise_smem_limit((const void*)forward_kernel<J, BMAX, MINB, MIXED, BURIED, GEN>, smem));
  int dev = 0, n_sm = 0, per_sm = 0;
  RFINV_CUDA_CHECK(cudaGetDevice(&dev));
  RFINV_CUDA_CHECK(cudaDeviceGetAttribute(&n_sm, cudaDevAttrMultiProcessorCount, dev));
  RFINV_CUDA_CHECK(cudaOccupancyMaxActiveBlocksPerMultiprocessor(&per_sm, forward_kernel<J, BMAX, MINB, MIXED, BURIED, GEN>, nthr, smem));
  if (per_sm < 1) { rfinv_set_error("forward_kernel does not fit on an SM (%zu bytes of shared memory)", smem); return RFINV_ERR_CUDA; }
  const int n_models = mb.active ? mb.n_active : mb.C;
  const long long items = (long long)n_models * sel.n;
  const long long resident = (long long)n_sm * per_sm;
  const unsigned grid = (unsigned)(items < resident ? items : resident);
  RFINV_CUDA_CHECK(rfinv_launch_pdl(1, forward_kernel<J, BMAX, MINB, MIXED, BURIED, GEN>, dim3(grid), dim3(nthr), smem, stream, cfg, mb, out, lc, rc, counter, sel));
  return RFINV_OK;
}

#ifndef RFINV_FWD_GENERAL_TU
}
int rfinv_launch_forward_group_general(const DevConfig& cfg, const ModelBatch& mb, const EvalOutputs& out, const double* lc,
                                       const double* rc, int* counter, int nthr, cudaStream_t stream, int sel_n,
                                       unsigned long long sel_packed);
namespace {
int launch_forward_group(const DevConfig& cfg, const ModelBatch& mb, const EvalOutputs& out, const double* lc, const double* rc,
                         int* counter, int nthr, cudaStream_t stream, const TraceSel& sel, int JB) {
  if (cfg.fft_general) return rfinv_launch_forward_group_general(cfg, mb, out, lc, rc, counter, nthr, stream, sel.n, sel.packed);
#define FWD(JJ, BB, MM)                                                                                   \
  do {                                                                                                    \
    if (cfg.bdep > 0.0) return launch_forward_t<JJ, BB, MM, true, true>(cfg, mb, out, lc, rc, counter, nthr, stream, sel); \
    if (JJ != JB) return launch_forward_t<JJ, BB, MM, true, false>(cfg, mb, out, lc, rc, counter, nthr, stream, sel); \
    return launch_forward_t<JJ, BB, MM, false, false>(cfg, mb, out, lc, rc, counter, nthr, stream, sel);  \
  } while (0)
  if (nthr <= 32) { if (JB <= 1) FWD(1, 32, 8); FWD(2, 32, 8); }
  if (nthr <= 64) { if (JB <= 2) FWD(2, 64, 6); FWD(4, 64, 6); }
  if (nthr <= 128) {
    if (JB <= 2) FWD(2, 128, 6);
    static const int minb3 = getenv("RFINV_FWD_MINB3") ? atoi(getenv("RFINV_FWD_MINB3")) : 4;
    if (JB <= 3) { if (minb3 == 5) FWD(3, 128, 5); FWD(3, 128, 4); }
    FWD(4, 128, 4);
  }
  if (JB <= 3) FWD(3, 256, 2);
  if (JB <= 4) FWD(4, 256, 2);
  if (JB <= 6) FWD(6, 256, 1);
  FWD(8, 256, 1);
#undef FWD
}
#endif

}

#ifdef RFINV_FWD_GENERAL_TU
int rfinv_launch_forward_group_general(const DevConfig& cfg, const ModelBatch& mb, const EvalOutputs& out, const double* lc,
                                       const double* rc, int* counter, int nthr, cudaStream_t stream, int sel_n,
                                       unsigned long long sel_packed) {
  TraceSel sel;
  sel.n = sel_n; sel.packed = sel_packed;
#define FWDG(JJ, BB, MM)                                                                                                \
  do {                                                                                                                  \
    if (cfg.bdep > 0.0) return launch_forward_t<JJ, BB, MM, true, true, true>(cfg, mb, out, lc, rc, counter, nthr, stream, sel); \
    return launch_forward_t<JJ, BB, MM, true, false, true>(cfg, mb, out, lc, rc, counter, nthr, stream, sel);           \
  } while (0)
  if (nthr <= 32) FWDG(2, 32, 8);
  if (nthr <= 64) FWDG(4, 64, 6);
  if (nthr <= 128) FWDG(4, 128, 4);
  FWDG(4, 256, 2);
#undef FWDG
}
#else

int rfinv_forward_bins_per_thread(int nfft) {
  if (nfft <= 64) return 1;
  if (nfft <= 256) return 2;
  if (nfft <= 2048) return 4;
  return 8;
}

size_t rfinv_forward_scratch_doubles(const DevConfig& cfg, long long n_models) {
  const long long ntr_eff = cfg.ray_common ? 1 : cfg.ntrc;
  return (size_t)(n_models * ntr_eff) * ((size_t)cfg.k_max * LC_DOUBLES + RC_DOUBLES) + RFINV_MAX_TRC / 2;
}

int rfinv_launch_prep(const DevConfig& cfg, const ModelBatch& mb, uint8_t* is_valid, double* scratch, cudaStream_t stream,
                      int m_begin, int m_count) {
  const int nthr = rfinv_forward_threads(cfg);
  const int n_models = mb.active ? mb.n_active : mb.C;
  const int ntr_eff = cfg.ray_common ? 1 : cfg.ntrc;
  const long long n_items = (long long)n_models * ntr_eff;
  if (m_count <= 0) return RFINV_OK;
  double* lc = scratch;
  double* rc = scratch + (size_t)n_items * cfg.k_max * LC_DOUBLES;
  int* counter = reinterpret_cast<int*>(rc + (size_t)n_items * RC_DOUBLES);
  int n_groups = 1;
  while (sizeof(double) * (prep_smem_model_doubles(cfg.k_max) + (size_t)((ntr_eff + n_groups - 1) / n_groups) * prep_smem_ray_doubles(cfg.k_max)) > 96 * 1024 &&
         n_groups < ntr_eff) ++n_groups;
  const int rays_per_cta = (ntr_eff + n_groups - 1) / n_groups;
  n_groups = (ntr_eff + rays_per_cta - 1) / rays_per_cta;
  const size_t prep_smem = sizeof(double) * (prep_smem_model_doubles(cfg.k_max) + (size_t)rays_per_cta * prep_smem_ray_doubles(cfg.k_max));
#define PREP(BUR, HOST)                                                                                                    \
  do {                                                                                                                     \
    RFINV_CUDA_CHECK(rfinv_raise_smem_limit((const void*)prep_kernel<BUR, HOST>, prep_smem));                                \
    prep_kernel<BUR, HOST><<<(unsigned)m_count * n_groups, 32 * rays_per_cta, prep_smem, stream>>>(cfg, mb, lc, rc, is_valid, counter, m_begin + m_count, ntr_eff, nthr, rays_per_cta, m_begin); \
  } while (0)
  if (cfg.bdep > 0.0) { if (mb.chain_major) PREP(true, true); else PREP(true, false); }
  else { if (mb.chain_major) PREP(false, true); else PREP(false, false); }
#undef PREP
  RFINV_CUDA_CHECK(cudaGetLastError());
  return RFINV_OK;
}

int rfinv_launch_forward(const DevConfig& cfg, const ModelBatch& mb, const EvalOutputs& out, double* scratch,
                         cudaStream_t stream, int* n_kernels, bool prep_done) {
  const int nthr = rfinv_forward_threads(cfg);
  const int n_models = mb.active ? mb.n_active : mb.C;
  const int ntr_eff = cfg.ray_common ? 1 : cfg.ntrc;
  const long long n_items = (long long)n_models * ntr_eff;
  if (n_items == 0) { if (n_kernels) *n_kernels = 0; return RFINV_OK; }
  double* lc = scratch;
  double* rc = scratch + (size_t)n_items * cfg.k_max * LC_DOUBLES;
  int* counter = reinterpret_cast<int*>(rc + (size_t)n_items * RC_DOUBLES);
  if (!prep_done) {
    const int st = rfinv_launch_prep(cfg, mb, out.is_valid, scratch, stream, 0, n_models);
    if (st != RFINV_OK) return st;
  }
  int n_launch = 0;
  for (int g = 8; g >= 1; --g) {
    TraceSel sel;
    sel.n = 0; sel.packed = 0ULL;
    if (cfg.ray_common) { if (g == cfg.jb_max) sel.push(0); }
    else for (int t = 0; t < cfg.ntrc; ++t) if (cfg.jbins[t] == g) sel.push(t);
    if (sel.n == 0) continue;
    const int st = launch_forward_group(cfg, mb, out, lc, rc, counter + n_launch, nthr, stream, sel, g);
    if (st != RFINV_OK) return st;
    ++n_launch;
  }
  if (n_kernels) *n_kernels = (prep_done ? 0 : 1) + n_launch;
  return RFINV_OK;
}

int rfinv_launch_filter_traces(const DevConfig& cfg, int n_series, const double* in, const int* trace_of, double* out,
                               cudaStream_t stream) {
  if (n_series == 0) return RFINV_OK;
  const size_t smem = sizeof(double2) * (2 * fft_buf_elems(cfg.fft_len) + (cfg.fft_general ? 0 : fft_twiddle_entries(cfg.fft_len))) + sizeof(double) * 64;
  const int nthr = cfg.fft_len / 8 < 32 ? 32 : (cfg.fft_len / 8 > 128 ? 128 : cfg.fft_len / 8);
  if (cfg.fft_general) {
    RFINV_CUDA_CHECK(rfinv_raise_smem_limit((const void*)filter_traces_kernel<true>, smem));
    filter_traces_kernel<true><<<n_series, nthr, smem, stream>>>(cfg, in, trace_of, out);
  } else {
    RFINV_CUDA_CHECK(rfinv_raise_smem_limit((const void*)filter_traces_kernel<false>, smem));
    filter_traces_kernel<false><<<n_series, nthr, smem, stream>>>(cfg, in, trace_of, out);
  }
  RFINV_CUDA_CHECK(cudaGetLastError());
  return RFINV_OK;
}

int rfinv_launch_format_model(const DevConfig& cfg, const ModelBatch& mb, int* nlay, double* alpha, double* beta,
                              double* rho, double* h, uint8_t* is_valid, cudaStream_t stream) {
  if (mb.C == 0) return RFINV_OK;
  format_model_kernel<<<(mb.C + 127) / 128, 128, 0, stream>>>(cfg, mb, nlay, alpha, beta, rho, h, is_valid);
  RFINV_CUDA_CHECK(cudaGetLastError());
  return RFINV_OK;
}
#endif
```

Before: 12.95 million.

## Restructure prep kernel to one warp per model with batched multi-ray layer passes

The prep kernel now maps one warp per model (four models per CTA) instead of one CTA per model with a warp per ray. Each warp sorts its own layers and then processes rays in passes of up to six, computing layer constants lane-parallel across layers. Interface scaling products for all rays in a pass are done by one batched warp scan, replacing the stored per-ray basis arrays. This removes block-wide syncs and the serial warp-0 setup phase while cutting shared memory per model. The cost is more registers per thread and more shuffles for each ray batch.

After: 13.42 million, median of 6. +3.6%, better.

```diff
diff --git a/rf_inv_b200/csrc/forward.cu b/rf_inv_b200/csrc/forward.cu
--- a/rf_inv_b200/csrc/forward.cu
+++ b/rf_inv_b200/csrc/forward.cu
@@ -158,25 +158,25 @@
   c[0] = c0; c[1] = c1; c[2] = c2; c[3] = c3;
 }
 
-struct PrepBasis {
-  double v14[4], v23[4];
-  double i14[4], i23[4];
-};
 struct PrepSerial {
   double tr[8];
   double ic[6];
-  double tpterm, pad;
+  double tpterm;
 };
 struct PrepShared {
   double h, rho, irho, beta2, inv_b2, inv_a2, a, b;
 };
-constexpr int PB_DOUBLES = sizeof(PrepBasis) / sizeof(double), PS_DOUBLES = sizeof(PrepSerial) / sizeof(double);
-constexpr int PSH_DOUBLES = sizeof(PrepShared) / sizeof(double);
+constexpr int PS_DOUBLES = sizeof(PrepSerial) / sizeof(double), PSH_DOUBLES = sizeof(PrepShared) / sizeof(double);
+constexpr int PREP_WARPS = 4;
 constexpr int PREP_RAYS_PER_PASS = 6;
-constexpr int PREP_MISC_DOUBLES = 8;
-__host__ __device__ inline size_t prep_sorted_doubles(int km) { return ((size_t)3 * km + 1) & ~(size_t)1; }
-__host__ __device__ inline size_t prep_smem_model_doubles(int km) { return prep_sorted_doubles(km) + (size_t)(km + 2) * PSH_DOUBLES + PREP_MISC_DOUBLES; }
-__host__ __device__ inline size_t prep_smem_ray_doubles(int km) { return (size_t)(km + 1) * PB_DOUBLES + (size_t)km * PS_DOUBLES + RC_DOUBLES + 8; }
+constexpr int PREP_CHAINS = 3;
+constexpr int PREP_WATER_DOUBLES = 8;
+__host__ __device__ inline size_t prep_ray_doubles(int km) {
+  return RC_DOUBLES + PREP_WATER_DOUBLES + (((size_t)km * PS_DOUBLES + 1) & ~(size_t)1);
+}
+__host__ __device__ inline size_t prep_warp_doubles(int km, int rays) {
+  return (size_t)(km + 1) * PSH_DOUBLES + (size_t)rays * prep_ray_doubles(km);
+}
 
 __device__ __forceinline__ void small_sincos(double x, double* sn, double* cs) {
   if (fabs(x) < 0.01) {
@@ -188,342 +188,407 @@
   }
 }
 
-__device__ __forceinline__ double warp_scan_mul(double x, int lane) {
+template <int N>
+__device__ __forceinline__ void warp_scan_mul(double (&x)[N], int lane) {
 #pragma unroll
   for (int o = 1; o < 32; o <<= 1) {
-    const double y = __shfl_up_sync(0xffffffffu, x, o);
-    if (lane >= o) x *= y;
-  }
-  return x;
+    double y[N];
+#pragma unroll
+    for (int i = 0; i < N; ++i) y[i] = __shfl_up_sync(0xffffffffu, x[i], o);
+#pragma unroll
+    for (int i = 0; i < N; ++i)
+      if (lane >= o) x[i] *= y[i];
+  }
+}
+
+__device__ __forceinline__ void prep_layer_ray(const PrepShared& S, double p2, double& bp, double& xi, double& eta) {
+  bp = 1.0 - 2.0 * S.beta2 * p2;
+  eta = sqrt(__dsub_rn(S.inv_b2, p2));
+  xi = sqrt(__dsub_rn(S.inv_a2, p2));
+}
+
+struct PrepRays {
+  const PrepShared* LA;
+  double* ray0;
+  size_t ray_stride;
+  LayerConst* lc0;
+  int t0;
+  int k, ka, kb, ls, nthr_fwd, nyq_doublings;
+};
+
+template <int R, bool BURIED>
+__device__ __forceinline__ void prep_rays(const DevConfig& cfg, const PrepRays& A, int lane) {
+  constexpr bool buried = BURIED;
+  const int k = A.k, ka = A.ka, kb = A.kb, ls = A.ls, km = cfg.k_max;
+  double p[R], p2[R];
+  int ipha[R];
+#pragma unroll
+  for (int r = 0; r < R; ++r) { p[r] = cfg.rayp[A.t0 + r]; ipha[r] = cfg.ipha[A.t0 + r]; p2[r] = __dmul_rn(p[r], p[r]); }
+  auto rec = [&](int r) { return reinterpret_cast<RayConst*>(A.ray0 + (size_t)r * A.ray_stride); };
+  auto water = [&](int r) { return A.ray0 + (size_t)r * A.ray_stride + RC_DOUBLES; };
+  auto serial = [&](int r) { return reinterpret_cast<PrepSerial*>(A.ray0 + (size_t)r * A.ray_stride + RC_DOUBLES + PREP_WATER_DOUBLES); };
+  const double nyq = (double)(cfg.nfft / 2);
+  double carryP[R], carryS[R];
+#pragma unroll
+  for (int r = 0; r < R; ++r) { carryP[r] = 1.0; carryS[r] = 1.0; }
+
+  for (int base = 0; base <= ka; base += 32) {
+    const int la = base + lane;
+    const PrepShared S = A.LA[la < ka ? la : ka];
+    const double h = S.h, rho = S.rho, beta2 = S.beta2;
+    double tp_sign = 1.0;
+    if (buried) {
+      if (la == ls) tp_sign = ls == k ? -1.0 : 0.0;
+      else if (la < ls) tp_sign = 0.0;
+    }
+    double bp[R], xi[R], eta[R];
+#pragma unroll
+    for (int r = 0; r < R; ++r) prep_layer_ray(S, p2[r], bp[r], xi[r], eta[r]);
+    if (la < ka) {
+#pragma unroll
+      for (int r = 0; r < R; ++r) {
+        PrepSerial& Z = serial(r)[la];
+        Z.tpterm = cfg.deconv_mode == 0 ? __dmul_rn(tp_sign, __dmul_rn(h, ipha[r] == 1 ? xi[r] : eta[r])) : 0.0;
+        LayerConst* L = A.lc0 + (size_t)r * km + la;
+        const double thx = cfg.domg * xi[r] * h, the = cfg.domg * eta[r] * h;
+        double snx, csx, sne, cse;
+        sincos(thx, &snx, &csx); L->c1x = csx; L->s1x = snx;
+        sincos(the, &sne, &cse); L->c1e = cse; L->s1e = sne;
+#pragma unroll
+        for (int d = 0; d < 4; ++d) {
+          const double c2 = fma(csx, csx, -snx * snx), s2 = 2.0 * csx * snx; csx = c2; snx = s2;
+          const double c3 = fma(cse, cse, -sne * sne), s3 = 2.0 * cse * sne; cse = c3; sne = s3;
+        }
+        L->c16x = csx; L->s16x = snx; L->c16e = cse; L->s16e = sne;
+        for (int b = 16; b < A.nthr_fwd; b <<= 1) {
+          const double c2 = fma(csx, csx, -snx * snx), s2 = 2.0 * csx * snx; csx = c2; snx = s2;
+          const double c3 = fma(cse, cse, -sne * sne), s3 = 2.0 * cse * sne; cse = c3; sne = s3;
+        }
+        L->cbx = csx; L->sbx = snx; L->cbe = cse; L->sbe = sne;
+        L->cb2x = csx + csx; L->cb2e = cse + cse;
+        small_sincos((double)1.0e-5f * xi[r] * h, &Z.tr[1], &Z.tr[0]);
+        small_sincos((double)1.0e-5f * eta[r] * h, &Z.tr[3], &Z.tr[2]);
+        double cn = csx, sn2 = snx, ce = cse, se = sne;
+        if (cfg.fft_general) {
+          sincos(nyq * thx, &sn2, &cn);
+          sincos(nyq * the, &se, &ce);
+        } else {
+          for (int d = 0; d < A.nyq_doublings; ++d) {
+            const double c2 = fma(cn, cn, -sn2 * sn2), s2 = 2.0 * cn * sn2; cn = c2; sn2 = s2;
+            const double c3 = fma(ce, ce, -se * se), s3 = 2.0 * ce * se; ce = c3; se = s3;
+          }
+        }
+        Z.tr[4] = cn; Z.tr[5] = sn2; Z.tr[6] = ce; Z.tr[7] = se;
+      }
+    } else if (la == ka) {
+#pragma unroll
+      for (int r = 0; r < R; ++r) { double* W = water(r); W[4] = xi[r]; W[5] = eta[r]; W[6] = bp[r]; }
+    }
+
+    double ieta[R];
+#pragma unroll
+    for (int r = 0; r < R; ++r) ieta[r] = 1.0 / eta[r];
+    double rho_n = __shfl_up_sync(0xffffffffu, rho, 1), beta2_n = __shfl_up_sync(0xffffffffu, beta2, 1);
+    double bp_n[R], xi_n[R], ieta_n[R];
+#pragma unroll
+    for (int r = 0; r < R; ++r) {
+      bp_n[r] = __shfl_up_sync(0xffffffffu, bp[r], 1);
+      xi_n[r] = __shfl_up_sync(0xffffffffu, xi[r], 1);
+      ieta_n[r] = __shfl_up_sync(0xffffffffu, ieta[r], 1);
+    }
+    if (lane == 0 && base > 0) {
+      const PrepShared N = A.LA[base - 1];
+      rho_n = N.rho; beta2_n = N.beta2;
+#pragma unroll
+      for (int r = 0; r < R; ++r) { double eta_n; prep_layer_ray(N, p2[r], bp_n[r], xi_n[r], eta_n); ieta_n[r] = 1.0 / eta_n; }
+    }
+    const bool iface = la >= 1 && la < ka;
+    auto basis = [&](int r, double* i14, double* i23, double* v14n, double* v23n) {
+      const double g2 = 2.0 * beta2 * p[r], irho = S.irho, ixi = 1.0 / xi[r];
+      const double g2n = 2.0 * beta2_n * p[r];
+      i14[0] = g2; i14[1] = irho; i14[2] = bp[r]; i14[3] = -p[r] * irho;
+      i23[0] = bp[r] * ixi; i23[1] = -p[r] * irho * ixi; i23[2] = -g2 * eta[r]; i23[3] = -eta[r] * irho;
+      v14n[0] = p[r]; v14n[1] = 1.0; v14n[2] = rho_n * bp_n[r]; v14n[3] = -rho_n * g2n;
+      v23n[0] = xi_n[r]; v23n[1] = -p[r] * ieta_n[r]; v23n[2] = -rho_n * g2n * xi_n[r]; v23n[3] = -rho_n * bp_n[r] * ieta_n[r];
+    };
+    double sc[2 * R];
+#pragma unroll
+    for (int r = 0; r < R; ++r) {
+      sc[2 * r] = 1.0; sc[2 * r + 1] = 1.0;
+      if (iface) {
+        double i14[4], i23[4], v14n[4], v23n[4];
+        basis(r, i14, i23, v14n, v23n);
+        sc[2 * r] = fma(i14[0], v14n[0], i14[1] * v14n[2]);
+        sc[2 * r + 1] = __dadd_rn(i14[2], __dmul_rn(i14[3], v14n[3]));
+      }
+    }
+    warp_scan_mul(sc, lane);
+#pragma unroll
+    for (int r = 0; r < R; ++r) {
+      const double sP = carryP[r] * sc[2 * r], sS = carryS[r] * sc[2 * r + 1];
+      double sPp = __shfl_up_sync(0xffffffffu, sP, 1), sSp = __shfl_up_sync(0xffffffffu, sS, 1);
+      if (lane == 0) { sPp = carryP[r]; sSp = carryS[r]; }
+      if (iface) {
+        double i14[4], i23[4], v14n[4], v23n[4], t23[4];
+        basis(r, i14, i23, v14n, v23n);
+        const double t14_1 = __dadd_rn(i14[0], __dmul_rn(i14[1], v14n[3]));
+        const double t14_2 = fma(i14[2], v14n[0], i14[3] * v14n[2]);
+        mat2_mul(i23, v23n, t23);
+        double* ic = serial(r)[la - 1].ic;
+        const double rP = 1.0 / sP, rS = 1.0 / sS;
+        const double pp = sPp * rP, sp = sSp * rP, ps = sPp * rS, ss = sSp * rS;
+        ic[0] = t14_1 * sp; ic[1] = t14_2 * ps;
+        ic[2] = t23[0] * pp; ic[3] = t23[1] * sp; ic[4] = t23[2] * ps; ic[5] = t23[3] * ss;
+        LayerConst* L = A.lc0 + (size_t)r * km + (la - 1);
+        L->t12 = ic[0]; L->t21 = ic[1]; L->u11 = ic[2]; L->u12 = ic[3]; L->u21 = ic[4]; L->u22 = ic[5];
+      }
+      RayConst* Rc = rec(r);
+      if (la == kb - 1) {
+        const double g2 = 2.0 * beta2 * p[r];
+        Rc->h14[0] = p[r] * sP; Rc->h14[1] = 1.0 * sS; Rc->h14[2] = rho * bp[r] * sP; Rc->h14[3] = -rho * g2 * sS;
+        Rc->h23[0] = xi[r] * sP; Rc->h23[1] = -p[r] * ieta[r] * sS; Rc->h23[2] = -rho * g2 * xi[r] * sP; Rc->h23[3] = -rho * bp[r] * ieta[r] * sS;
+      }
+      if (la == 0) {
+        const double g2 = 2.0 * beta2 * p[r], irho = S.irho, ixi = 1.0 / xi[r];
+        Rc->a1 = g2; Rc->b1 = bp[r];
+        Rc->q1a = irho; Rc->q1b = -p[r] * irho;
+        Rc->q2a = bp[r] * ixi; Rc->q2b = -g2 * eta[r];
+      }
+      if (buried && la == ls) {
+        Rc->sta[0] = p[r] * sP; Rc->sta[1] = 1.0 * sS;
+        Rc->sta[2] = xi[r] * sP; Rc->sta[3] = -p[r] * ieta[r] * sS;
+      }
+      const int last_lane = (ka - 1 - base) < 31 ? (ka - 1 - base) : 31;
+      carryP[r] = __shfl_sync(0xffffffffu, sP, last_lane);
+      carryS[r] = __shfl_sync(0xffffffffu, sS, last_lane);
+    }
+  }
+  if (lane < R) {
+#pragma unroll
+    for (int r = 0; r < R; ++r) {
+      if (r != lane) continue;
+      LayerConst* L = A.lc0 + (size_t)r * km + (ka - 1);
+      L->t12 = 0.0; L->t21 = 0.0; L->u11 = 1.0; L->u12 = 0.0; L->u21 = 0.0; L->u22 = 1.0;
+      double* ic = serial(r)[ka - 1].ic;
+      ic[0] = 0.0; ic[1] = 0.0; ic[2] = 1.0; ic[3] = 0.0; ic[4] = 0.0; ic[5] = 1.0;
+    }
+  }
 }
 
 template <bool BURIED, bool HOSTLAYOUT>
-__global__ void __maxnreg__(80) prep_kernel(const DevConfig cfg, const ModelBatch mb, double* __restrict__ lc_out,
+__global__ void __launch_bounds__(32 * PREP_WARPS, 4) prep_kernel(const DevConfig cfg, const ModelBatch mb, double* __restrict__ lc_out,
                                                                  double* __restrict__ rc_out, uint8_t* __restrict__ is_valid,
                                                                  int* __restrict__ counter, int n_models, int ntr_eff, int nthr_fwd,
-                                                                 int rays_per_cta, int m_begin) {
+                                                                 int rays_per_pass, int m_begin) {
   extern __shared__ __align__(16) double prep_smem[];
   const int warp = threadIdx.x >> 5, lane = threadIdx.x & 31;
-  const int n_groups = (ntr_eff + rays_per_cta - 1) / rays_per_cta;
-  const int bm = blockIdx.x / n_groups, t_first = (blockIdx.x - bm * n_groups) * rays_per_cta;
-  const int ci = m_begin + bm;
-  const int nr_cta = min(rays_per_cta, ntr_eff - t_first);
+  const int ci = m_begin + blockIdx.x * PREP_WARPS + warp;
   pdl_trigger();
   if (blockIdx.x == 0 && m_begin == 0 && threadIdx.x < RFINV_MAX_TRC) counter[threadIdx.x] = 0;
   if (ci >= n_models) return;
   if (mb.n_active_dev && ci >= *mb.n_active_dev) return;
   const int c = mb.active ? mb.active[ci] : ci;
   const int km = cfg.k_max, C = mb.C;
-  const bool has_ray = warp < nr_cta;
-  const int t0 = t_first + (has_ray ? warp : 0);
-  const size_t item = (size_t)ci * ntr_eff + t0;
-  double* zs = prep_smem;
+  PrepShared* LA = reinterpret_cast<PrepShared*>(prep_smem + (size_t)warp * prep_warp_doubles(km, rays_per_pass));
+  double* ray0 = reinterpret_cast<double*>(LA + km + 1);
+  const size_t ray_stride = prep_ray_doubles(km);
+  auto ray_const = [&](int r) { return reinterpret_cast<RayConst*>(ray0 + (size_t)r * ray_stride); };
+  auto ray_water = [&](int r) { return ray0 + (size_t)r * ray_stride + RC_DOUBLES; };
+  auto ray_serial = [&](int r) { return reinterpret_cast<const PrepSerial*>(ray0 + (size_t)r * ray_stride + RC_DOUBLES + PREP_WATER_DOUBLES); };
+  constexpr bool buried = BURIED;
+
+  PREP_INIT();
+  int k = mb.k[c];
+  double zr[2] = {0.0, 0.0}, dr[2] = {0.0, 0.0}, sr[2] = {0.0, 0.0};
+  static_assert(RFINV_MAX_K <= 64, "two elements per lane");
+#pragma unroll
+  for (int q = 0; q < 2; ++q) {
+    const int i = lane + 32 * q;
+    if (i < km - 1) {
+      if (HOSTLAYOUT) {
+        zr[q] = mb.z[(size_t)c * (km - 1) + i]; sr[q] = mb.dvs[(size_t)c * km + i];
+        if (cfg.vp_mode == 1) dr[q] = mb.dvp[(size_t)c * km + i];
+      } else {
+        zr[q] = mb.z[(size_t)i * C + c]; dr[q] = mb.dvp[(size_t)i * C + c]; sr[q] = mb.dvs[(size_t)i * C + c];
+      }
+    }
+  }
+  double dvs_half, dvp_half = 0.0;
+  if (HOSTLAYOUT) { dvs_half = mb.dvs[(size_t)c * km + km - 1]; if (cfg.vp_mode == 1) dvp_half = mb.dvp[(size_t)c * km + km - 1]; }
+  else { dvs_half = mb.dvs[(size_t)(km - 1) * C + c]; dvp_half = mb.dvp[(size_t)(km - 1) * C + c]; }
+  k = k < 1 ? 1 : (k > km - 1 ? km - 1 : k);
+  double* zs = ray0;
   double *dps = zs + km, *dss = dps + km;
-  PrepShared* LA = reinterpret_cast<PrepShared*>(zs + prep_sorted_doubles(km));
-  double* s_misc = reinterpret_cast<double*>(LA + km + 2);
-  int* s_int = reinterpret_cast<int*>(s_misc + 1);
-  double* ray0 = s_misc + PREP_MISC_DOUBLES;
-  const size_t ray_stride = prep_smem_ray_doubles(km);
-  auto ray_basis = [&](int t) { return reinterpret_cast<PrepBasis*>(ray0 + (size_t)t * ray_stride); };
-  auto ray_serial = [&](int t) { return reinterpret_cast<PrepSerial*>(ray0 + (size_t)t * ray_stride + (size_t)(km + 1) * PB_DOUBLES); };
-  auto ray_const = [&](int t) { return reinterpret_cast<RayConst*>(ray0 + (size_t)t * ray_stride + (size_t)(km + 1) * PB_DOUBLES + (size_t)km * PS_DOUBLES); };
-  auto ray_water = [&](int t) { return reinterpret_cast<double*>(ray_const(t)) + RC_DOUBLES; };
-  constexpr bool buried = BURIED;
-
-  PREP_INIT();
-  if (warp == 0) {
-    int k = mb.k[c];
-    double zr[2] = {0.0, 0.0}, dr[2] = {0.0, 0.0}, sr[2] = {0.0, 0.0};
-    static_assert(RFINV_MAX_K <= 64, "two elements per lane");
-#pragma unroll
-    for (int q = 0; q < 2; ++q) {
-      const int i = lane + 32 * q;
-      if (i < km - 1) {
-        if (HOSTLAYOUT) {
-          zr[q] = mb.z[(size_t)c * (km - 1) + i]; sr[q] = mb.dvs[(size_t)c * km + i];
-          if (cfg.vp_mode == 1) dr[q] = mb.dvp[(size_t)c * km + i];
-        } else {
-          zr[q] = mb.z[(size_t)i * C + c]; dr[q] = mb.dvp[(size_t)i * C + c]; sr[q] = mb.dvs[(size_t)i * C + c];
-        }
-      }
-    }
-    double dvs_half, dvp_half = 0.0;
-    if (HOSTLAYOUT) { dvs_half = mb.dvs[(size_t)c * km + km - 1]; if (cfg.vp_mode == 1) dvp_half = mb.dvp[(size_t)c * km + km - 1]; }
-    else { dvs_half = mb.dvs[(size_t)(km - 1) * C + c]; dvp_half = mb.dvp[(size_t)(km - 1) * C + c]; }
-    k = k < 1 ? 1 : (k > km - 1 ? km - 1 : k);
-    double* zu = reinterpret_cast<double*>(ray_basis(0));
-    double *du = zu + km, *su = du + km;
-#pragma unroll
-    for (int q = 0; q < 2; ++q) {
-      const int i = lane + 32 * q;
-      if (i < k) { zu[i] = zr[q]; du[i] = dr[q]; su[i] = sr[q]; }
-    }
-    __syncwarp();
-    for (int i = lane; i < k; i += 32) {
-      const double zi = zu[i];
-      int rank = 0;
-      for (int j = 0; j < k; ++j) { const double zj = zu[j]; rank += (zj < zi || (zj == zi && j < i)) ? 1 : 0; }
-      zs[rank] = zi; dps[rank] = du[i]; dss[rank] = su[i];
-    }
-    __syncwarp();
-
-    int ls = -1;
-    double h_part = 0.0;
+  double* zu = dss + km;
+  double *du = zu + km, *su = du + km;
+#pragma unroll
+  for (int q = 0; q < 2; ++q) {
+    const int i = lane + 32 * q;
+    if (i < k) { zu[i] = zr[q]; du[i] = dr[q]; su[i] = sr[q]; }
+  }
+  __syncwarp();
+  for (int i = lane; i < k; i += 32) {
+    const double zi = zu[i];
+    int rank = 0;
+    for (int j = 0; j < k; ++j) { const double zj = zu[j]; rank += (zj < zi || (zj == zi && j < i)) ? 1 : 0; }
+    zs[rank] = zi; dps[rank] = du[i]; dss[rank] = su[i];
+  }
+  __syncwarp();
+
+  int ls = -1;
+  double h_part = 0.0;
+  if (buried) {
+    double z_tmp = 0.0;
+    ls = k;
+    for (int l = 0; l < k; ++l) {
+      const double hl = l == 0 ? __dsub_rn(zs[0], cfg.sdep) : __dsub_rn(zs[l], zs[l - 1]);
+      z_tmp = __dadd_rn(z_tmp, hl);
+      if (!(z_tmp < cfg.bdep)) { ls = l; h_part = __dsub_rn(__dadd_rn(cfg.bdep, hl), z_tmp); break; }
+    }
+    if (ls == k) h_part = __dsub_rn(cfg.bdep, z_tmp);
+  }
+  const int ka = buried ? k + 1 : k;
+  PREP_MARK(0);
+  bool valid = true;
+  for (int la = lane; la <= ka; la += 32) {
+    const int l = (buried && la > ls) ? la - 1 : la;
+    double zc, h, dvs_l, dvp_l;
+    if (l == 0) { zc = __dmul_rn(0.5, __dadd_rn(cfg.sdep, zs[0])); h = __dsub_rn(zs[0], cfg.sdep); dvs_l = dss[0]; dvp_l = dps[0]; }
+    else if (l < k) { zc = __dmul_rn(0.5, __dadd_rn(zs[l], zs[l - 1])); h = __dsub_rn(zs[l], zs[l - 1]); dvs_l = dss[l]; dvp_l = dps[l]; }
+    else { zc = __dmul_rn(0.5, __dadd_rn(cfg.z_max, zs[k - 1])); h = 999.0; dvs_l = dvs_half; dvp_l = dvp_half; }
+    double a, b;
+    bool ok = layer_velocity(cfg, zc, dvs_l, dvp_l, a, b);
+    if (l == 0) ok = ok && !(h < __dmul_rn(0.125, a));
+    else if (l < k) ok = ok && !(h < cfg.h_min);
+    valid = valid && ok;
     if (buried) {
-      double z_tmp = 0.0;
-      ls = k;
-      for (int l = 0; l < k; ++l) {
-        const double hl = l == 0 ? __dsub_rn(zs[0], cfg.sdep) : __dsub_rn(zs[l], zs[l - 1]);
-        z_tmp = __dadd_rn(z_tmp, hl);
-        if (!(z_tmp < cfg.bdep)) { ls = l; h_part = __dsub_rn(__dadd_rn(cfg.bdep, hl), z_tmp); break; }
-      }
-      if (ls == k) h_part = __dsub_rn(cfg.bdep, z_tmp);
-    }
-    const int ka = buried ? k + 1 : k;
-    PREP_MARK(0);
-    bool valid = true;
-    for (int la = lane; la <= ka; la += 32) {
-      const int l = (buried && la > ls) ? la - 1 : la;
-      double zc, h, dvs_l, dvp_l;
-      if (l == 0) { zc = __dmul_rn(0.5, __dadd_rn(cfg.sdep, zs[0])); h = __dsub_rn(zs[0], cfg.sdep); dvs_l = dss[0]; dvp_l = dps[0]; }
-      else if (l < k) { zc = __dmul_rn(0.5, __dadd_rn(zs[l], zs[l - 1])); h = __dsub_rn(zs[l], zs[l - 1]); dvs_l = dss[l]; dvp_l = dps[l]; }
-      else { zc = __dmul_rn(0.5, __dadd_rn(cfg.z_max, zs[k - 1])); h = 999.0; dvs_l = dvs_half; dvp_l = dvp_half; }
-      double a, b;
-      bool ok = layer_velocity(cfg, zc, dvs_l, dvp_l, a, b);
-      if (l == 0) ok = ok && !(h < __dmul_rn(0.125, a));
-      else if (l < k) ok = ok && !(h < cfg.h_min);
-      valid = valid && ok;
-      if (buried) {
-        if (la == ls) h = h_part;
-        else if (la == ls + 1 && ls < k) h = __dsub_rn(h, h_part);
-      }
-      PrepShared S;
-      S.h = h; S.a = a; S.b = b;
-      S.rho = vp_to_rho(a);
-      S.irho = 1.0 / S.rho;
-      S.beta2 = __dmul_rn(b, b);
-      S.inv_b2 = __ddiv_rn(1.0, S.beta2);
-      S.inv_a2 = __ddiv_rn(1.0, __dmul_rn(a, a));
-      LA[la] = S;
-    }
-    valid = __all_sync(0xffffffffu, valid);
-    if (lane == 0) { s_int[0] = k; s_int[1] = ls; s_int[2] = valid ? 1 : 0; s_misc[0] = h_part; }
-    PREP_MARK(1);
-  }
-  __syncthreads();
-
-  const int k = s_int[0], ls = s_int[1];
-  const bool valid = s_int[2] != 0;
-  const int ka = buried ? k + 1 : k;
+      if (la == ls) h = h_part;
+      else if (la == ls + 1 && ls < k) h = __dsub_rn(h, h_part);
+    }
+    PrepShared S;
+    S.h = h; S.a = a; S.b = b;
+    S.rho = vp_to_rho(a);
+    S.irho = 1.0 / S.rho;
+    S.beta2 = __dmul_rn(b, b);
+    S.inv_b2 = __ddiv_rn(1.0, S.beta2);
+    S.inv_a2 = __ddiv_rn(1.0, __dmul_rn(a, a));
+    LA[la] = S;
+  }
+  valid = __all_sync(0xffffffffu, valid);
+  __syncwarp();
+  PREP_MARK(1);
+
   const int kb = (buried && ls == k) ? k : ka;
-  PrepBasis* PB = ray_basis(warp);
-  PrepSerial* PS = ray_serial(warp);
-  if (has_ray) {
-
-  const double p = cfg.rayp[t0];
-  const int ipha = cfg.ipha[t0];
-  const double p2 = __dmul_rn(p, p);
-  const double nyq = (double)(cfg.nfft / 2);
   int nyq_doublings = 0;
   while ((nthr_fwd << nyq_doublings) < cfg.nfft_p2 / 2) ++nyq_doublings;
-  for (int la = lane; la <= ka; la += 32) {
-    const PrepShared S = LA[la];
-    const double h = S.h, rho = S.rho, beta2 = S.beta2;
-    double tp_sign = 1.0;
-    if (buried) {
-      if (la == ls) tp_sign = ls == k ? -1.0 : 0.0;
-      else if (la < ls) tp_sign = 0.0;
-    }
-    const double bp = 1.0 - 2.0 * beta2 * p2;
-    const double eta = sqrt(__dsub_rn(S.inv_b2, p2));
-    const double xi = sqrt(__dsub_rn(S.inv_a2, p2));
-    if (la < ka) {
-      PrepBasis& Q = PB[la];
-      PrepSerial& Z = PS[la];
-      const double g2 = 2.0 * beta2 * p;
-      const double ieta = 1.0 / eta, irho = S.irho, ixi = 1.0 / xi;
-      Q.v14[0] = p; Q.v14[1] = 1.0; Q.v14[2] = rho * bp; Q.v14[3] = -rho * g2;
-      Q.v23[0] = xi; Q.v23[1] = -p * ieta; Q.v23[2] = -rho * g2 * xi; Q.v23[3] = -rho * bp * ieta;
-      Q.i14[0] = g2; Q.i14[1] = irho; Q.i14[2] = bp; Q.i14[3] = -p * irho;
-      Q.i23[0] = bp * ixi; Q.i23[1] = -p * irho * ixi; Q.i23[2] = -g2 * eta; Q.i23[3] = -eta * irho;
-      Z.tpterm = cfg.deconv_mode == 0 ? __dmul_rn(tp_sign, __dmul_rn(h, ipha == 1 ? xi : eta)) : 0.0;
-      LayerConst* L = reinterpret_cast<LayerConst*>(lc_out) + item * km + la;
-      const double thx = cfg.domg * xi * h, the = cfg.domg * eta * h;
-      double snx, csx, sne, cse;
-      sincos(thx, &snx, &csx); L->c1x = csx; L->s1x = snx;
-      sincos(the, &sne, &cse); L->c1e = cse; L->s1e = sne;
-#pragma unroll
-      for (int d = 0; d < 4; ++d) {
-        const double c2 = fma(csx, csx, -snx * snx), s2 = 2.0 * csx * snx; csx = c2; snx = s2;
-        const double c3 = fma(cse, cse, -sne * sne), s3 = 2.0 * cse * sne; cse = c3; sne = s3;
-      }
-      L->c16x = csx; L->s16x = snx; L->c16e = cse; L->s16e = sne;
-      for (int b = 16; b < nthr_fwd; b <<= 1) {
-        const double c2 = fma(csx, csx, -snx * snx), s2 = 2.0 * csx * snx; csx = c2; snx = s2;
-        const double c3 = fma(cse, cse, -sne * sne), s3 = 2.0 * cse * sne; cse = c3; sne = s3;
-      }
-      L->cbx = csx; L->sbx = snx; L->cbe = cse; L->sbe = sne;
-      L->cb2x = csx + csx; L->cb2e = cse + cse;
-      small_sincos((double)1.0e-5f * xi * h, &Z.tr[1], &Z.tr[0]);
-      small_sincos((double)1.0e-5f * eta * h, &Z.tr[3], &Z.tr[2]);
-      double cn = csx, sn2 = snx, ce = cse, se = sne;
-      if (cfg.fft_general) {
-        sincos(nyq * thx, &sn2, &cn);
-        sincos(nyq * the, &se, &ce);
+  for (int t_first = 0; t_first < ntr_eff; t_first += rays_per_pass) {
+    const int nr = min(rays_per_pass, ntr_eff - t_first);
+    const size_t item = (size_t)ci * ntr_eff + t_first;
+    for (int r0 = 0; r0 < nr; r0 += PREP_CHAINS) {
+      PrepRays A;
+      A.LA = LA; A.ray0 = ray0 + (size_t)r0 * ray_stride; A.ray_stride = ray_stride;
+      A.lc0 = reinterpret_cast<LayerConst*>(lc_out) + (item + r0) * km; A.t0 = t_first + r0;
+      A.k = k; A.ka = ka; A.kb = kb; A.ls = ls; A.nthr_fwd = nthr_fwd; A.nyq_doublings = nyq_doublings;
+      static_assert(PREP_CHAINS == 3, "sub-batches of 1 to 3 rays");
+      const int nb = min(PREP_CHAINS, nr - r0);
+      if (nb == 3) prep_rays<3, BURIED>(cfg, A, lane);
+      else if (nb == 2) prep_rays<2, BURIED>(cfg, A, lane);
+      else prep_rays<1, BURIED>(cfg, A, lane);
+    }
+    __syncwarp();
+    PREP_MARK(2);
+
+    if (lane < nr) {
+      const double p = cfg.rayp[t_first + lane];
+      RayConst* R = ray_const(lane);
+      double* W = ray_water(lane);
+      const double nyq = (double)(cfg.nfft / 2);
+      double cw0 = 1.0, sw0 = 0.0, cw1 = 1.0, sw1 = 0.0, rw = 0.0;
+      if (cfg.sdep > 0.0) {
+        const double aw = 1.5, rhow = 1.0, hw = cfg.sdep;
+        const double xiw = sqrt(1.0 / (aw * aw) - p * p);
+        const double thw = cfg.domg * xiw * hw;
+        double ws[4], cbw, sbw;
+        sincos(thw, &ws[1], &ws[0]);
+        cbw = ws[0]; sbw = ws[1];
+#pragma unroll
+        for (int d = 0; d < 4; ++d) { const double c2 = fma(cbw, cbw, -sbw * sbw), s2 = 2.0 * cbw * sbw; cbw = c2; sbw = s2; }
+        ws[2] = cbw; ws[3] = sbw;
+        for (int b = 16; b < nthr_fwd; b <<= 1) { const double c2 = fma(cbw, cbw, -sbw * sbw), s2 = 2.0 * cbw * sbw; cbw = c2; sbw = s2; }
+        R->thw = thw; R->cbw = cbw; R->sbw = sbw;
+        R->wseed[0] = ws[0]; R->wseed[1] = ws[1]; R->wseed[2] = ws[2]; R->wseed[3] = ws[3];
+        rw = rhow / xiw;
+        small_sincos((double)1.0e-5f * xiw * hw, &sw0, &cw0);
+        sincos(nyq * thw, &sw1, &cw1);
       } else {
-        for (int d = 0; d < nyq_doublings; ++d) {
-          const double c2 = fma(cn, cn, -sn2 * sn2), s2 = 2.0 * cn * sn2; cn = c2; sn2 = s2;
-          const double c3 = fma(ce, ce, -se * se), s3 = 2.0 * ce * se; ce = c3; se = s3;
+        R->thw = 0.0; R->cbw = 1.0; R->sbw = 0.0;
+        R->wseed[0] = R->wseed[2] = 1.0; R->wseed[1] = R->wseed[3] = 0.0;
+      }
+      {
+        const PrepShared& H = LA[ka];
+        const double a = H.a, b = H.b, rho = H.rho, beta2 = H.beta2, xi = W[4], eta = W[5], bp = W[6];
+        const double r1 = 1.0 / (2.0 * rho * a * xi), r2 = 1.0 / (2.0 * rho * b * eta);
+        const double e11 = beta2 * p * (2.0 * rho * xi) * r1, e12 = bp * rho * r1, e13 = p * r1, e14 = xi * r1;
+        const double e21 = bp * rho * r2, e22 = b * p, e23 = eta * r2, e24 = p * r2;
+        const double r14[4] = {e11, e14, e21, -e24};
+        const double r23[4] = {-e12, e13, e22, e23};
+        const double v14[4] = {R->h14[0], R->h14[1], R->h14[2], R->h14[3]};
+        const double v23[4] = {R->h23[0], R->h23[1], R->h23[2], R->h23[3]};
+        double h14[4], h23[4];
+        mat2_mul(r14, v14, h14);
+        mat2_mul(r23, v23, h23);
+#pragma unroll
+        for (int i = 0; i < 4; ++i) { R->h14[i] = h14[i]; R->h23[i] = h23[i]; }
+      }
+      R->q1a = -rw * R->q1a; R->q1b = -rw * R->q1b;
+      if (buried) R->l_sta = ls;
+      else { R->l_sta = -1; R->sta[0] = R->sta[1] = R->sta[2] = R->sta[3] = 0.0; }
+      R->k = kb;
+      R->valid = valid;
+      R->tp = 0.0; R->npre = 0;
+#pragma unroll
+      for (int i = 0; i < 4; ++i) R->edge[i] = make_double2(0.0, 0.0);
+      W[0] = cw0; W[1] = sw0; W[2] = cw1; W[3] = sw1;
+    }
+    __syncwarp();
+    PREP_MARK(3);
+
+    {
+      const bool vec_lane = lane < 4 * nr, tp_lane = lane >= 4 * nr && lane < 5 * nr;
+      const int tr_ray = vec_lane ? (lane >> 2) : (tp_lane ? lane - 4 * nr : 0);
+      const RayConst* Rr = ray_const(tr_ray);
+      const double* Wr = ray_water(tr_ray);
+      const PrepSerial* Zr = ray_serial(tr_ray);
+      const bool is_b = lane & 1, is_nyq = (lane >> 1) & 1;
+      Wave w;
+      double2 y_sta = make_double2(0.0, 0.0);
+      double tp = 0.0;
+      {
+        const double cw = is_nyq ? Wr[2] : Wr[0], sw = is_nyq ? Wr[3] : Wr[1];
+        if (!is_b) { w.a1 = Rr->a1; w.b1 = Rr->b1; w.a2 = 0.0; w.b2 = 0.0; }
+        else { w.a1 = sw * Rr->q1a; w.b1 = sw * Rr->q1b; w.a2 = cw * Rr->q2a; w.b2 = cw * Rr->q2b; }
+      }
+      if (vec_lane) {
+        const int o = is_nyq ? 4 : 0;
+        const double st0 = Rr->sta[0], st1 = Rr->sta[1], st2 = Rr->sta[2], st3 = Rr->sta[3];
+        Wave w_bc = w;
+        for (int l = 0; l < ka; ++l) {
+          const PrepSerial& Q = Zr[l];
+          wave_rotate(w, Q.tr[o], Q.tr[o + 1], Q.tr[o + 2], Q.tr[o + 3]);
+          if (buried && l == ls) { y_sta.x = fma(st0, w.a1, st1 * w.b1); y_sta.y = fma(st2, w.a2, st3 * w.b2); }
+          if (l == kb - 1) w_bc = w;
+          if (l + 1 < ka) wave_interface(w, Q.ic[0], Q.ic[1], Q.ic[2], Q.ic[3], Q.ic[4], Q.ic[5]);
         }
-      }
-      Z.tr[4] = cn; Z.tr[5] = sn2; Z.tr[6] = ce; Z.tr[7] = se;
-    } else {
-      double* W = ray_water(warp);
-      W[4] = xi; W[5] = eta; W[6] = bp;
-    }
-  }
-  __syncwarp();
-
-  PREP_MARK(2);
-  double carryP = 1.0, carryS = 1.0;
-  double sP_last = 1.0, sS_last = 1.0;
-  double sP_sta = 1.0, sS_sta = 1.0;
-  for (int base = 0; base < ka; base += 32) {
-    const int l = base + lane;
-    double t14[4] = {1.0, 0.0, 0.0, 1.0}, t23[4] = {1.0, 0.0, 0.0, 1.0};
-    if (l >= 1 && l < ka) {
-      mat2_mul(PB[l].i14, PB[l - 1].v14, t14);
-      mat2_mul(PB[l].i23, PB[l - 1].v23, t23);
-    }
-    const double sP = carryP * warp_scan_mul(t14[0], lane), sS = carryS * warp_scan_mul(t14[3], lane);
-    double sPp = __shfl_up_sync(0xffffffffu, sP, 1), sSp = __shfl_up_sync(0xffffffffu, sS, 1);
-    if (lane == 0) { sPp = carryP; sSp = carryS; }
-    if (l >= 1 && l < ka) {
-      double* ic = PS[l - 1].ic;
-      const double rP = 1.0 / sP, rS = 1.0 / sS;
-      const double pp = sPp * rP, sp = sSp * rP, ps = sPp * rS, ss = sSp * rS;
-      ic[0] = t14[1] * sp; ic[1] = t14[2] * ps;
-      ic[2] = t23[0] * pp; ic[3] = t23[1] * sp; ic[4] = t23[2] * ps; ic[5] = t23[3] * ss;
-      LayerConst* L = reinterpret_cast<LayerConst*>(lc_out) + item * km + (l - 1);
-      L->t12 = ic[0]; L->t21 = ic[1]; L->u11 = ic[2]; L->u12 = ic[3]; L->u21 = ic[4]; L->u22 = ic[5];
-    }
-    const int last_lane = (ka - 1 - base) < 31 ? (ka - 1 - base) : 31;
-    if (buried && ls >= base && ls < base + 32) { sP_sta = __shfl_sync(0xffffffffu, sP, ls - base); sS_sta = __shfl_sync(0xffffffffu, sS, ls - base); }
-    if (kb - 1 >= base && kb - 1 < base + 32) { sP_last = __shfl_sync(0xffffffffu, sP, kb - 1 - base); sS_last = __shfl_sync(0xffffffffu, sS, kb - 1 - base); }
-    carryP = __shfl_sync(0xffffffffu, sP, last_lane);
-    carryS = __shfl_sync(0xffffffffu, sS, last_lane);
-  }
-  if (lane == 0) {
-    LayerConst* L = reinterpret_cast<LayerConst*>(lc_out) + item * km + (ka - 1);
-    L->t12 = 0.0; L->t21 = 0.0; L->u11 = 1.0; L->u12 = 0.0; L->u21 = 0.0; L->u22 = 1.0;
-    double* ic = PS[ka - 1].ic;
-    ic[0] = 0.0; ic[1] = 0.0; ic[2] = 1.0; ic[3] = 0.0; ic[4] = 0.0; ic[5] = 1.0;
-  }
-  __syncwarp();
-
-  PREP_MARK(3);
-  {
-    RayConst R;
-    double cw0 = 1.0, sw0 = 0.0, cw1 = 1.0, sw1 = 0.0, rw = 0.0;
-    if (cfg.sdep > 0.0) {
-      const double aw = 1.5, rhow = 1.0, hw = cfg.sdep;
-      const double xiw = sqrt(1.0 / (aw * aw) - p * p);
-      R.thw = cfg.domg * xiw * hw;
-      sincos(R.thw, &R.wseed[1], &R.wseed[0]);
-      R.cbw = R.wseed[0]; R.sbw = R.wseed[1];
-#pragma unroll
-      for (int d = 0; d < 4; ++d) { const double c2 = fma(R.cbw, R.cbw, -R.sbw * R.sbw), s2 = 2.0 * R.cbw * R.sbw; R.cbw = c2; R.sbw = s2; }
-      R.wseed[2] = R.cbw; R.wseed[3] = R.sbw;
-      for (int b = 16; b < nthr_fwd; b <<= 1) { const double c2 = fma(R.cbw, R.cbw, -R.sbw * R.sbw), s2 = 2.0 * R.cbw * R.sbw; R.cbw = c2; R.sbw = s2; }
-      rw = rhow / xiw;
-      small_sincos((double)1.0e-5f * xiw * hw, &sw0, &cw0);
-      sincos(nyq * R.thw, &sw1, &cw1);
-    } else {
-      R.thw = 0.0; R.cbw = 1.0; R.sbw = 0.0;
-      R.wseed[0] = R.wseed[2] = 1.0; R.wseed[1] = R.wseed[3] = 0.0;
-    }
-    {
-      const PrepShared& H = LA[ka];
-      const double* W = ray_water(warp);
-      const double a = H.a, b = H.b, rho = H.rho, beta2 = H.beta2, xi = W[4], eta = W[5], bp = W[6];
-      const double r1 = 1.0 / (2.0 * rho * a * xi), r2 = 1.0 / (2.0 * rho * b * eta);
-      const double e11 = beta2 * p * (2.0 * rho * xi) * r1, e12 = bp * rho * r1, e13 = p * r1, e14 = xi * r1;
-      const double e21 = bp * rho * r2, e22 = b * p, e23 = eta * r2, e24 = p * r2;
-      const double r14[4] = {e11, e14, e21, -e24};
-      const double r23[4] = {-e12, e13, e22, e23};
-      const PrepBasis& Q = PB[kb - 1];
-      const double v14[4] = {Q.v14[0] * sP_last, Q.v14[1] * sS_last, Q.v14[2] * sP_last, Q.v14[3] * sS_last};
-      const double v23[4] = {Q.v23[0] * sP_last, Q.v23[1] * sS_last, Q.v23[2] * sP_last, Q.v23[3] * sS_last};
-      mat2_mul(r14, v14, R.h14);
-      mat2_mul(r23, v23, R.h23);
-    }
-    {
-      const PrepBasis& Q = PB[0];
-      R.a1 = Q.i14[0]; R.b1 = Q.i14[2];
-      R.q1a = -rw * Q.i14[1]; R.q1b = -rw * Q.i14[3];
-      R.q2a = Q.i23[0]; R.q2b = Q.i23[2];
-    }
-    R.l_sta = -1;
-    R.sta[0] = R.sta[1] = R.sta[2] = R.sta[3] = 0.0;
-    if (buried) {
-      const PrepBasis& Q = PB[ls];
-      R.l_sta = ls;
-      R.sta[0] = Q.v14[0] * sP_sta; R.sta[1] = Q.v14[1] * sS_sta;
-      R.sta[2] = Q.v23[0] * sP_sta; R.sta[3] = Q.v23[1] * sS_sta;
-    }
-    R.k = kb;
-    R.valid = valid;
-    R.tp = 0.0; R.npre = 0;
-#pragma unroll
-    for (int i = 0; i < 4; ++i) R.edge[i] = make_double2(0.0, 0.0);
-    if (lane == 0) {
-      *ray_const(warp) = R;
-      double* W = ray_water(warp);
-      W[0] = cw0; W[1] = sw0; W[2] = cw1; W[3] = sw1;
-    }
-  }
-  PREP_MARK(4);
-  }
-  __syncthreads();
-
-  for (int r0 = warp * PREP_RAYS_PER_PASS; r0 < nr_cta; r0 += (int)(blockDim.x >> 5) * PREP_RAYS_PER_PASS) {
-    const int nr = min(PREP_RAYS_PER_PASS, nr_cta - r0);
-    const bool vec_lane = lane < 4 * nr, tp_lane = lane >= 4 * nr && lane < 5 * nr;
-    const int tr_ray = r0 + (vec_lane ? (lane >> 2) : (tp_lane ? lane - 4 * nr : 0));
-    const RayConst* Rr = ray_const(tr_ray);
-    const double* Wr = ray_water(tr_ray);
-    const PrepSerial* Zr = ray_serial(tr_ray);
-    const bool is_b = lane & 1, is_nyq = (lane >> 1) & 1;
-    Wave w;
-    double2 y_sta = make_double2(0.0, 0.0);
-    double tp = 0.0;
-    {
-      const double cw = is_nyq ? Wr[2] : Wr[0], sw = is_nyq ? Wr[3] : Wr[1];
-      if (!is_b) { w.a1 = Rr->a1; w.b1 = Rr->b1; w.a2 = 0.0; w.b2 = 0.0; }
-      else { w.a1 = sw * Rr->q1a; w.b1 = sw * Rr->q1b; w.a2 = cw * Rr->q2a; w.b2 = cw * Rr->q2b; }
-    }
-    if (vec_lane) {
-      const int o = is_nyq ? 4 : 0;
-      const double st0 = Rr->sta[0], st1 = Rr->sta[1], st2 = Rr->sta[2], st3 = Rr->sta[3];
-      Wave w_bc = w;
-      for (int l = 0; l < ka; ++l) {
-        const PrepSerial& Q = Zr[l];
-        wave_rotate(w, Q.tr[o], Q.tr[o + 1], Q.tr[o + 2], Q.tr[o + 3]);
-        if (buried && l == ls) { y_sta.x = fma(st0, w.a1, st1 * w.b1); y_sta.y = fma(st2, w.a2, st3 * w.b2); }
-        if (l == kb - 1) w_bc = w;
-        if (l + 1 < ka) wave_interface(w, Q.ic[0], Q.ic[1], Q.ic[2], Q.ic[3], Q.ic[4], Q.ic[5]);
-      }
-      w = w_bc;
-    } else if (tp_lane) {
-      for (int l = 0; l < ka; ++l) tp = __dadd_rn(tp, Zr[l].tpterm);
-      RayConst* Rw = ray_const(tr_ray);
-      const int iph = cfg.ipha[t_first + tr_ray];
-      Rw->tp = tp;
-      Rw->npre = iph == 1 ? f_nint((-cfg.t_start - tp) / cfg.delta)
-                          : f_nint((-cfg.t_start + tp) / cfg.delta);
-    }
-    PREP_MARK(5);
-    {
+        w = w_bc;
+      } else if (tp_lane) {
+        for (int l = 0; l < ka; ++l) tp = __dadd_rn(tp, Zr[l].tpterm);
+        RayConst* Rw = ray_const(tr_ray);
+        const int iph = cfg.ipha[t_first + tr_ray];
+        Rw->tp = tp;
+        Rw->npre = iph == 1 ? f_nint((-cfg.t_start - tp) / cfg.delta)
+                            : f_nint((-cfg.t_start + tp) / cfg.delta);
+      }
+      PREP_MARK(4);
       const int rr = lane >> 1, e = lane & 1;
       const bool fin = lane < 2 * nr;
       const int src_a = fin ? 4 * rr + 2 * e : 0, src_b = src_a + 1;
@@ -535,28 +600,29 @@
       const double2 ya = make_double2(__shfl_sync(0xffffffffu, y_sta.x, src_a), __shfl_sync(0xffffffffu, y_sta.y, src_a));
       const double2 yb = make_double2(__shfl_sync(0xffffffffu, y_sta.x, src_b), __shfl_sync(0xffffffffu, y_sta.y, src_b));
       if (fin) {
-        RayConst* Rf = ray_const(r0 + rr);
-        const double* Wf = ray_water(r0 + rr);
+        RayConst* Rf = ray_const(rr);
+        const double* Wf = ray_water(rr);
         double h14[4], h23[4];
 #pragma unroll
         for (int i = 0; i < 4; ++i) { h14[i] = Rf->h14[i]; h23[i] = Rf->h23[i]; }
         double2 fr, fv;
-        if (!buried) surface_response(h14, h23, ea, eb, e ? Wf[2] : Wf[0], cfg.ipha[t_first + r0 + rr], fr, fv);
-        else surface_response_buried(h14, h23, ea, eb, cfg.ipha[t_first + r0 + rr], ya, yb, fr, fv);
+        if (!buried) surface_response(h14, h23, ea, eb, e ? Wf[2] : Wf[0], cfg.ipha[t_first + rr], fr, fv);
+        else surface_response_buried(h14, h23, ea, eb, cfg.ipha[t_first + rr], ya, yb, fr, fv);
         Rf->edge[2 * e] = fr; Rf->edge[2 * e + 1] = fv;
       }
     }
-  }
-  __syncthreads();
-  {
-    double2* dst = reinterpret_cast<double2*>(rc_out + ((size_t)ci * ntr_eff + t_first) * RC_DOUBLES);
-    for (int i = threadIdx.x; i < nr_cta * (RC_DOUBLES / 2); i += blockDim.x) {
-      const int t = i / (RC_DOUBLES / 2), j = i - t * (RC_DOUBLES / 2);
-      dst[i] = reinterpret_cast<const double2*>(ray_const(t))[j];
-    }
-    if (is_valid && threadIdx.x == 0 && t_first == 0) is_valid[c] = (uint8_t)valid;
-  }
-  PREP_MARK(6);
+    __syncwarp();
+    {
+      double2* dst = reinterpret_cast<double2*>(rc_out + item * RC_DOUBLES);
+      for (int i = lane; i < nr * (RC_DOUBLES / 2); i += 32) {
+        const int t = i / (RC_DOUBLES / 2), j = i - t * (RC_DOUBLES / 2);
+        dst[i] = reinterpret_cast<const double2*>(ray_const(t))[j];
+      }
+      if (is_valid && lane == 0 && t_first == 0) is_valid[c] = (uint8_t)valid;
+    }
+    __syncwarp();
+    PREP_MARK(5);
+  }
 }
 
 __host__ __device__ inline size_t fft_twiddle_entries(size_t n) {
@@ -1479,16 +1545,13 @@
   double* lc = scratch;
   double* rc = scratch + (size_t)n_items * cfg.k_max * LC_DOUBLES;
   int* counter = reinterpret_cast<int*>(rc + (size_t)n_items * RC_DOUBLES);
-  int n_groups = 1;
-  while (sizeof(double) * (prep_smem_model_doubles(cfg.k_max) + (size_t)((ntr_eff + n_groups - 1) / n_groups) * prep_smem_ray_doubles(cfg.k_max)) > 96 * 1024 &&
-         n_groups < ntr_eff) ++n_groups;
-  const int rays_per_cta = (ntr_eff + n_groups - 1) / n_groups;
-  n_groups = (ntr_eff + rays_per_cta - 1) / rays_per_cta;
-  const size_t prep_smem = sizeof(double) * (prep_smem_model_doubles(cfg.k_max) + (size_t)rays_per_cta * prep_smem_ray_doubles(cfg.k_max));
+  const int rays_per_pass = ntr_eff < PREP_RAYS_PER_PASS ? ntr_eff : PREP_RAYS_PER_PASS;
+  const size_t prep_smem = sizeof(double) * PREP_WARPS * prep_warp_doubles(cfg.k_max, rays_per_pass);
+  const unsigned n_cta = (unsigned)((m_count + PREP_WARPS - 1) / PREP_WARPS);
 #define PREP(BUR, HOST)                                                                                                    \
   do {                                                                                                                     \
     RFINV_CUDA_CHECK(rfinv_raise_smem_limit((const void*)prep_kernel<BUR, HOST>, prep_smem));                                \
-    prep_kernel<BUR, HOST><<<(unsigned)m_count * n_groups, 32 * rays_per_cta, prep_smem, stream>>>(cfg, mb, lc, rc, is_valid, counter, m_begin + m_count, ntr_eff, nthr, rays_per_cta, m_begin); \
+    prep_kernel<BUR, HOST><<<n_cta, 32 * PREP_WARPS, prep_smem, stream>>>(cfg, mb, lc, rc, is_valid, counter, m_begin + m_count, ntr_eff, nthr, rays_per_pass, m_begin); \
   } while (0)
   if (cfg.bdep > 0.0) { if (mb.chain_major) PREP(true, true); else PREP(true, false); }
   else { if (mb.chain_major) PREP(false, true); else PREP(false, false); }
```
